# actionml/universal-recommender

Measured on NVIDIA H100. Metric: CCO train events/sec to indicator model, higher is better.
Workload: dtype int32+f64

## Files before the change

### universal_recommender_b200/csrc/cco_api.cu

```cuda
#include <cuda_runtime.h>
#include <dlfcn.h>
#include <stdarg.h>
#include <stdio.h>
#include <stdlib.h>
#include <string.h>

#include <algorithm>
#include <cmath>
#include <functional>
#include <cub/cub.cuh>
#include <nvtx3/nvToolsExt.h>
#include <condition_variable>
#include <mutex>
#include <string>
#include <thread>
#include <unordered_map>
#include <vector>

#include "../../include/cco_b200.h"
#include "cco_kernels.cuh"
#include "cco_sampler.cuh"
#include "cco_format.cuh"
#include "cco_strings.cuh"
#include "cco_json.cuh"
// ... 150 lines not shown
      return pinned[best].p;
    }
    void *p = nullptr;
    size_t cap = (bytes + (1u << 20) - 1) & ~((size_t)(1u << 20) - 1);
    if (cudaHostAlloc(&p, cap, cudaHostAllocPortable) != cudaSuccess) return nullptr;
    pinned.push_back({p, cap, true});
    return p;
  }
  void pinned_put(void *p) {
    std::lock_guard<std::mutex> lk(mu);
    if (arena && (unsigned char *)p >= arena && (unsigned char *)p < arena + arena_bytes) {
      if (--arena_live <= 0) { arena_live = 0; arena_used = 0; }
      return;
    }
    for (auto &b : pinned)
      if (b.p == p) b.used = false;
  }
};

struct ResultMat {
  int64_t row_begin = 0, row_end = 0;
  int32_t n_cols = 0;
  int64_t *row_ptr = nullptr;
  int32_t *col = nullptr;
  double *llr = nullptr;
  int32_t *cnt = nullptr;
};
struct cco_dataset {
  cco_ctx *ctx = nullptr;
  int n_mats = 0;
  long long n_users = 0;
  long long row_base = 0, n_local = 0;
  std::vector<long long> n_cols, nnz;
  std::vector<long long *> rp;
  std::vector<int32_t *> col;
  std::vector<void *> rp_alloc, col_alloc;
  std::vector<long long> block_cap;
  std::vector<long long> q_lo, q_hi;
  std::vector<cudaEvent_t> ready;
  bool h2d_pending = false;
  bool validated = false;
  bool whole = false;
  float ms_h2d = 0;
  std::vector<cco_dictionary_t> dicts;
};

struct cco_result {
  cco_ctx *ctx = nullptr;
  std::vector<ResultMat> mats;
  cco_stats_t stats;
};

namespace cco {

struct Arena {
  cudaStream_t s;
  cco_ctx *c;
  std::vector<void *> ptrs;
  static constexpr size_t kSlabMax = 8u << 20, kSlabBytes = 64u << 20;
  explicit Arena(cudaStream_t st, cco_ctx *ctx = nullptr) : s(st), c(ctx && !ctx->slab_busy ? ctx : nullptr) {
    if (c) {
      c->slab_busy = true;
      c->slab_idx = 0;
      c->slab_off = 0;
    }
  }
  ~Arena() {
    for (void *p : ptrs) cudaFreeAsync(p, s);
    if (c) c->slab_busy = false;
  }
  void *bump(size_t bytes) {
    bytes = (bytes + 255) & ~(size_t)255;
    while (true) {
      if (c->slab_idx < c->slabs.size()) {
        cco_ctx::Slab &sl = c->slabs[c->slab_idx];
        if (c->slab_off + bytes <= sl.cap) {
          void *p = sl.p + c->slab_off;
          c->slab_off += bytes;
          return p;
        }
        ++c->slab_idx;
        c->slab_off = 0;
        continue;
      }
      void *p = nullptr;
      if (cudaMalloc(&p, kSlabBytes) != cudaSuccess) return nullptr;
      c->slabs.push_back({(unsigned char *)p, kSlabBytes});
    }
  }
  template <typename T>
  int alloc(T **out, size_t n) {
    void *p = nullptr;
    size_t bytes = std::max<size_t>(n * sizeof(T), 16);
    if (c && bytes <= kSlabMax) {
      p = bump(bytes);
      if (!p) return set_error(CCO_E_OOM, "cudaMalloc(scratch slab) failed");
      *out = (T *)p;
      return CCO_OK;
    }
    cudaError_t e = cudaMallocAsync(&p, bytes, s);
    if (e != cudaSuccess) return set_error(CCO_E_OOM, "cudaMallocAsync(%zu bytes): %s", bytes, cudaGetErrorString(e));
    ptrs.push_back(p);
    *out = (T *)p;
    return CCO_OK;
  }
  void take(void *p) {
    for (size_t i = 0; i < ptrs.size(); ++i)
      if (ptrs[i] == p) {
        ptrs.erase(ptrs.begin() + i);
        return;
      }
  }
  void release(void *p) {
    for (size_t i = 0; i < ptrs.size(); ++i)
      if (ptrs[i] == p) {
        cudaFreeAsync(p, s);
        ptrs.erase(ptrs.begin() + i);
        return;
      }
  }
};
static int pooled_event(cco_ctx *c, bool timing, cudaEvent_t *out) {
  std::vector<cudaEvent_t> &pool = timing ? c->ev_timing : c->ev_plain;
  size_t &used = timing ? c->ev_timing_used : c->ev_plain_used;
  if (used == pool.size()) {
    cudaEvent_t e;
    CK(timing ? cudaEventCreate(&e) : cudaEventCreateWithFlags(&e, cudaEventDisableTiming));
    pool.push_back(e);
  }
  *out = pool[used++];
  return CCO_OK;
}

static inline void nvtx_push(const char *name) { nvtxRangePushA(name); }
static inline void nvtx_pop() { nvtxRangePop(); }

static inline int grid_for(long long work_items, int block, int sm_count, int waves = 8) {
  long long g = (work_items + block - 1) / block;
  long long cap = (long long)sm_count * waves;
  if (g > cap) g = cap;
  if (g < 1) g = 1;
  return (int)g;
}

constexpr size_t kMailBytes = 1 << 16;
static int mail_fetch(cco_ctx *c, void *dst_host, const void *src_dev, size_t n) {
  size_t off = (c->mail_used + 7) & ~(size_t)7;
  if (off + n > kMailBytes) return set_error(CCO_E_CUDA, "internal: mailbox overflow");
  k_mail_bytes<<<1, 128, 0, c->stream>>>(c->mail_d + off, (const unsigned char *)src_dev, (int)n);
  c->mail_pending.push_back({dst_host, off, n, c->mail_group});
  c->mail_used = off + n;
  return CCO_OK;
}
static int mail_close(cco_ctx *c, int *group) {
  const int g = c->mail_group;
  while ((int)c->mail_ev.size() <= g) {
    cudaEvent_t e;
    CK(cudaEventCreateWithFlags(&e, cudaEventDisableTiming));
    c->mail_ev.push_back(e);
  }
  CK(cudaEventRecord(c->mail_ev[g], c->stream));
  c->mail_group = g + 1;
  if (group) *group = g;
  return CCO_OK;
}
static int mail_wait_group(cco_ctx *c, int g) {
  CK(cudaEventSynchronize(c->mail_ev[g]));
  CK(cudaGetLastError());
  for (auto &m : c->mail_pending)
    if (m.group == g) memcpy(m.dst, c->mail_h + m.off, m.n);
  return CCO_OK;
}
static void mail_reset(cco_ctx *c) {
  c->mail_pending.clear();
  c->mail_used = 0;
  c->mail_group = 0;
}
static int mail_wait(cco_ctx *c) {
  int g = 0;
  CKR(mail_close(c, &g));
  return mail_wait_group(c, g);
}

struct DevRaw {
  long long n_rows = 0;
  long long row_base = 0;
  int32_t n_cols = 0;
  long long nnz = 0;
  long long nnz_cap = 0;
  long long q_base = 0;
  long long *rp = nullptr;
  int32_t *col = nullptr;
};
struct DevMat {
  long long n_rows = 0;
  int32_t n_cols = 0;
  uint32_t *rp = nullptr;
  int32_t *col = nullptr;
  int32_t *marg = nullptr;
};

template <typename T>
static int exclusive_sum(cco_ctx *c, Arena &ar, const T *in, T *out, long long n, cudaStream_t on = nullptr) {
  if (!on) on = c->stream;
  size_t tb = 0;
  CK(cub::DeviceScan::ExclusiveSum(nullptr, tb, in, out, n, on));
  void *tmp;
  CKR(ar.alloc((char **)&tmp, tb));
  CK(cub::DeviceScan::ExclusiveSum(tmp, tb, in, out, n, on));
  ar.release(tmp);
  return CCO_OK;
}
template <typename K, typename V>
static int sort_pairs(cco_ctx *c, Arena &ar, long long n, K **k, V **v, int bits) {
  cudaStream_t s = c->stream;
  K *k1;
  V *v1;
  CKR(ar.alloc(&k1, std::max<long long>(n, 1)));
  CKR(ar.alloc(&v1, std::max<long long>(n, 1)));
  cub::DoubleBuffer<K> kb(*k, k1);
  cub::DoubleBuffer<V> vb(*v, v1);
  size_t tbytes = 0;
  CK(cub::DeviceRadixSort::SortPairs(nullptr, tbytes, kb, vb, n, 0, bits, s));
  void *tmp;
  CKR(ar.alloc((char **)&tmp, tbytes));
  CK(cub::DeviceRadixSort::SortPairs(tmp, tbytes, kb, vb, n, 0, bits, s));
  c->launches++;
  ar.release(tmp);
  ar.release(kb.Alternate());
  ar.release(vb.Alternate());
  *k = kb.Current();
  *v = vb.Current();
  return CCO_OK;
}
static int bits_for(long long n) {
  int b = 1;
  while ((1LL << b) < n) ++b;
  return b;
}

static int canonicalize_device(cco_ctx *c, Arena &ar, DevRaw &m) {
  if (m.nnz == 0) return CCO_OK;
  unsigned long long *k0, *k1;
  CKR(ar.alloc(&k0, m.nnz));
  CKR(ar.alloc(&k1, m.nnz));
  k_expand_keys<<<grid_for(m.n_rows * kSG, 256, c->sm_count), 256, 0, c->stream>>>(m.n_rows, m.rp, m.col, k0);
  c->launches++;
  int row_bits = 1;
  while ((1LL << row_bits) < m.n_rows) ++row_bits;
  cub::DoubleBuffer<unsigned long long> db(k0, k1);
  size_t tb = 0;
  CK(cub::DeviceRadixSort::SortKeys(nullptr, tb, db, m.nnz, 0, 32 + row_bits, c->stream));
  void *tmp;
  CKR(ar.alloc((char **)&tmp, tb));
  CK(cub::DeviceRadixSort::SortKeys(tmp, tb, db, m.nnz, 0, 32 + row_bits, c->stream));
  ar.release(tmp);
  unsigned long long *sorted = db.Current(), *other = db.Alternate();
  uint32_t *flag, *pos;
  CKR(ar.alloc(&flag, m.nnz + 1));
  CKR(ar.alloc(&pos, m.nnz + 1));
  CK(cudaMemsetAsync(flag + m.nnz, 0, 4, c->stream));
  k_unique_flags<<<grid_for(m.nnz, 256, c->sm_count), 256, 0, c->stream>>>(m.nnz, sorted, flag);
  c->launches++;
  CKR(exclusive_sum(c, ar, flag, pos, m.nnz + 1));
  uint32_t n_unique = 0;
  CK(cudaMemcpyAsync(&n_unique, pos + m.nnz, 4, cudaMemcpyDeviceToHost, c->stream));
  k_unique_scatter<<<grid_for(m.nnz, 256, c->sm_count), 256, 0, c->stream>>>(m.nnz, sorted, flag, pos, other, m.col + m.q_base);
  CK(cudaStreamSynchronize(c->stream));
  k_rowptr_from_keys<<<grid_for(m.n_rows + 1, 256, c->sm_count), 256, 0, c->stream>>>(m.n_rows, n_unique, other, m.rp);
  c->launches += 2;
  m.col += m.q_base;
  m.q_base = 0;
  m.nnz = n_unique;
  CK(cudaGetLastError());
  ar.release(flag);
  ar.release(pos);
  ar.release(k0);
  ar.release(k1);
  return CCO_OK;
}

struct HeavyRows {
  int32_t *list = nullptr;
  int *n = nullptr;
};
static int list_heavy_rows(cco_ctx *c, Arena &ar, const DevRaw &raw, HeavyRows *h) {
  CKR(ar.alloc(&h->list, std::max<long long>(raw.n_rows, 1)));
  CKR(ar.alloc(&h->n, 1));
  CK(cudaMemsetAsync(h->n, 0, 4, c->stream));
  if (raw.n_rows > 0) {
    k_list_heavy_rows<<<grid_for(raw.n_rows, 256, c->sm_count), 256, 0, c->stream>>>(raw.n_rows, raw.rp, h->list, h->n);
    c->launches++;
  }
  return CCO_OK;
}
static void launch_check(cco_ctx *c, const DevRaw &raw, const HeavyRows &h, int *flags) {
  if (raw.n_rows <= 0) return;
  const long long q_lo = raw.q_base, q_hi = raw.q_base + raw.nnz;
  k_check_rows<kSG><<<grid_for(raw.n_rows * kSG, 256, c->sm_count), 256, 0, c->stream>>>(raw.n_rows, raw.n_cols, raw.rp, raw.col, q_lo, q_hi,
                                                                                       nullptr, nullptr, flags);
  k_check_rows<32><<<c->sm_count * 4, 256, 0, c->stream>>>(raw.n_rows, raw.n_cols, raw.rp, raw.col, q_lo, q_hi, h.list, h.n, flags);
  c->launches += 2;
}
struct SampleScratch {
  unsigned long long *col_thr = nullptr;
  uint8_t *keep = nullptr;
};
static int sample_scratch(cco_ctx *c, Arena &ar, const DevRaw &raw, const int32_t *raw_counts, int32_t m, SampleScratch *sc) {
  CKR(ar.alloc(&sc->col_thr, std::max<int32_t>(raw.n_cols, 1)));
  CKR(ar.alloc(&sc->keep, std::max<long long>(raw.nnz, 1)));
  if (raw.n_cols > 0) {
    k_col_thresholds<<<grid_for(raw.n_cols, 256, c->sm_count, 4), 256, 0, c->stream>>>(raw.n_cols, raw_counts, m, sc->col_thr);
    c->launches++;
  }
  return CCO_OK;
}
static void launch_count(cco_ctx *c, const DevRaw &raw, const SampleScratch &sc, int32_t m, int32_t seed, uint32_t flags, const int *bad,
                         uint32_t *kept, int32_t *new_counts) {
  if (raw.n_rows <= 0 || raw.nnz <= 0) return;
  const long long q_lo = raw.q_base, q_hi = raw.q_base + raw.nnz;
  const long long n_chunks = (raw.nnz + kSampleChunk - 1) / kSampleChunk;
  k_sample_count<<<grid_for(n_chunks * 32, 256, c->sm_count), 256, 0, c->stream>>>(raw.n_rows, raw.row_base, raw.rp, raw.col, raw.n_cols, q_lo, q_hi,
                                                                                  sc.col_thr, m, seed, flags, bad, kept, new_counts, sc.keep);
  c->launches++;
}
static int launch_write(cco_ctx *c, Arena &ar, const DevRaw &raw, const SampleScratch &sc, int32_t *dst) {
  if (raw.n_rows <= 0 || raw.nnz <= 0) return CCO_OK;
  long long *n_sel;
  CKR(ar.alloc(&n_sel, 1));
  size_t tb = 0;
  CK(cub::DeviceSelect::Flagged(nullptr, tb, raw.col + raw.q_base, sc.keep, dst, n_sel, (long long)raw.nnz, c->stream));
  void *tmp;
  CKR(ar.alloc((char **)&tmp, tb));
  CK(cub::DeviceSelect::Flagged(tmp, tb, raw.col + raw.q_base, sc.keep, dst, n_sel, (long long)raw.nnz, c->stream));
  ar.release(tmp);
  c->launches += 2;
  return CCO_OK;
}

constexpr int kHistCopies = 16;
static int count_raw_columns(cco_ctx *c, const std::vector<DevRaw> &raw, const std::vector<long long> &col_off, const cudaEvent_t *ready,
                             int *verdict, int32_t *counts) {
  cudaStream_t s = c->stream;
  const int n_mats = (int)raw.size();
  const long long total_cols = col_off[n_mats];
  const long long copy_stride = std::max<long long>(total_cols, 1);
  for (int i = 0; i < n_mats; ++i) {
    if (ready) CK(cudaStreamWaitEvent(s, ready[i], 0));
    if (raw[i].n_rows == 0) continue;
    int *v = verdict ? verdict + 2 * i : nullptr;
    if (v) {
      k_check_row_ptr<<<grid_for(raw[i].n_rows, 256, c->sm_count), 256, 0, s>>>(raw[i].n_rows, raw[i].rp, raw[i].q_base, raw[i].q_base + raw[i].nnz, v);
      c->launches++;
    }
    if (raw[i].nnz > 0) {
      k_col_histogram_flat<true><<<grid_for(raw[i].nnz, 256, c->sm_count), 256, 0, s>>>(raw[i].nnz, raw[i].col + raw[i].q_base, raw[i].n_cols,
                                                                                       counts + col_off[i], kHistCopies, copy_stride, v);
      c->launches++;
    }
  }
  if (total_cols > 0) {
    k_sum_copies<<<grid_for(total_cols, 256, c->sm_count), 256, 0, s>>>(total_cols, kHistCopies, copy_stride, counts);
    c->launches++;
  }
  return CCO_OK;
}

static int downsample_device(cco_ctx *c, Arena &ar, const DevRaw &raw, const int *bad, const int32_t *raw_counts, int32_t m,
                             int32_t seed, uint32_t flags, DevMat *out) {
  out->n_rows = raw.n_rows;
  out->n_cols = raw.n_cols;
  uint32_t *kept;
  CKR(ar.alloc(&kept, raw.n_rows + 1));
  CKR(ar.alloc(&out->rp, raw.n_rows + 1));
  if (!out->marg) CKR(ar.alloc(&out->marg, std::max<int32_t>(raw.n_cols, 1)));
  CKR(ar.alloc(&out->col, std::max<long long>(raw.nnz, 1)));
  CK(cudaMemsetAsync(out->marg, 0, sizeof(int32_t) * std::max<int32_t>(raw.n_cols, 1), c->stream));
  CK(cudaMemsetAsync(kept, 0, sizeof(uint32_t) * ((size_t)raw.n_rows + 1), c->stream));
  SampleScratch sc;
  CKR(sample_scratch(c, ar, raw, raw_counts, m, &sc));
  launch_count(c, raw, sc, m, seed, flags, bad, kept, out->marg);
  CKR(exclusive_sum(c, ar, kept, out->rp, raw.n_rows + 1));
  CKR(launch_write(c, ar, raw, sc, out->col));
  CK(cudaGetLastError());
  ar.release(kept);
  ar.release(sc.col_thr);
  ar.release(sc.keep);
  return CCO_OK;
}

static int nccl_check(int rc, const char *what) {
  if (rc != 0) return set_error(CCO_E_NCCL, "%s: %s", what, g_nccl.GetErrorString(rc));
  return CCO_OK;
}

static int downsample_sharded_all(cco_ctx *c, Arena &ar, const std::vector<DevRaw> &raw, const int *d_check ,
                                  const std::vector<long long> &block_cap,
                                  long long U, const int32_t *raw_counts, int32_t *marg_all, const std::vector<long long> &col_off,
                                  const cco_indicator_params_t *params, int32_t seed, uint32_t flags, std::vector<DevMat> &dm,
                                  cudaEvent_t *stage_ev ) {
  cudaStream_t s = c->stream;
  const int W = c->world, r = c->rank, n_mats = (int)raw.size();
  const long long S = (U + W - 1) / W;
  const long long row_base = raw[0].row_base;
  std::vector<uint32_t *> kept(n_mats, nullptr);
  std::vector<SampleScratch> sc(n_mats);
  for (int i = 0; i < n_mats; ++i) {
    DevMat *out = &dm[i];
    out->n_rows = U;
    out->n_cols = raw[i].n_cols;
    out->marg = marg_all + col_off[i];
    CKR(ar.alloc(&kept[i], (size_t)(W * S + 1)));
    CKR(ar.alloc(&out->rp, U + 1));
    CK(cudaMemsetAsync(kept[i], 0, sizeof(uint32_t) * (size_t)(W * S + 1), s));
    CKR(sample_scratch(c, ar, raw[i], raw_counts + col_off[i], params[i].max_interactions, &sc[i]));
    launch_count(c, raw[i], sc[i], params[i].max_interactions, seed, flags, d_check + 2 * i, kept[i], out->marg);
  }
  CK(cudaEventRecord(stage_ev[0], s));
  if (S > 0) {
    g_nccl.GroupStart();
    for (int i = 0; i < n_mats; ++i) {
      int rc = g_nccl.AllGather(kept[i] + (size_t)r * S, kept[i], (size_t)S, kNcclUint32, c->comm, s);
      if (rc != 0) { g_nccl.GroupEnd(); return nccl_check(rc, "ncclAllGather(kept counts)"); }
    }
    CKR(nccl_check(g_nccl.GroupEnd(), "ncclGroupEnd(kept counts)"));
  }
  if (col_off[n_mats] > 0)
    CKR(nccl_check(g_nccl.AllReduce(marg_all, marg_all, (size_t)col_off[n_mats], kNcclInt32, kNcclSum, c->comm, s), "ncclAllReduce(marginals)"));
  std::vector<int32_t *> gathered(n_mats, nullptr);
  std::vector<uint32_t> edge((size_t)n_mats * (W + 1), 0);
  for (int i = 0; i < n_mats; ++i) {
    CKR(exclusive_sum(c, ar, kept[i], dm[i].rp, U + 1));
    ar.release(kept[i]);
    for (int q = 0; q <= W; ++q) CKR(mail_fetch(c, &edge[(size_t)i * (W + 1) + q], dm[i].rp + std::min<long long>((long long)q * S, U), 4));
  }
  CK(cudaEventRecord(stage_ev[1], s));
  CKR(mail_wait(c));
  std::vector<long long> cap(n_mats, 0);
  for (int i = 0; i < n_mats; ++i) {
    for (int q = 0; q < W; ++q) cap[i] = std::max<long long>(cap[i], (long long)edge[(size_t)i * (W + 1) + q + 1] - edge[(size_t)i * (W + 1) + q]);
    CKR(ar.alloc(&dm[i].col, std::max<long long>(edge[(size_t)i * (W + 1) + W], 1)));
    if (cap[i] == 0) continue;
    CKR(ar.alloc(&gathered[i], (size_t)(cap[i] * W)));
    CKR(launch_write(c, ar, raw[i], sc[i], gathered[i] + (size_t)r * cap[i]));
    ar.release(sc[i].col_thr);
    ar.release(sc[i].keep);
  }
  CK(cudaEventRecord(stage_ev[2], s));
  g_nccl.GroupStart();
  for (int i = 0; i < n_mats; ++i) {
    if (!gathered[i]) continue;
    int rc = g_nccl.AllGather(gathered[i] + (size_t)r * cap[i], gathered[i], (size_t)cap[i], kNcclInt32, c->comm, s);
    if (rc != 0) { g_nccl.GroupEnd(); return nccl_check(rc, "ncclAllGather(column blocks)"); }
  }
  CKR(nccl_check(g_nccl.GroupEnd(), "ncclGroupEnd(column blocks)"));
  for (int i = 0; i < n_mats; ++i) {
    if (!gathered[i]) continue;
    dim3 grid((unsigned)std::max(1, std::min(c->sm_count * 8 / W, 1024)), (unsigned)W);
    k_pack_blocks<<<grid, 256, 0, s>>>(W, S, U, cap[i], dm[i].rp, gathered[i], dm[i].col);
    c->launches++;
    ar.release(gathered[i]);
  }
  CK(cudaEventRecord(stage_ev[3], s));
  CK(cudaGetLastError());
  return CCO_OK;
}


struct BinCfg {
  int group;
  int slots;
  int cap;
  int cbuf;
  int caux, keep_max, final_max;
  bool dense;
  bool bitmap;
  int bm_words;
  size_t region;
  size_t smem;
  int ctas_per_sm;
};

static int next_pow2(int x) {
  int p = 1;
  while (p < x) p <<= 1;
  return p;
}

template <int GROUP>
static int launch_rows_t(cco_ctx *c, const RowArgs &a, BinCfg &cfg, cudaStream_t st) {
  constexpr int CTA = GROUP == 32 ? 64 : GROUP;
  int occ = 1;
  void (*kern)(const RowArgs) = cfg.dense ? k_rows<GROUP, true> : k_rows<GROUP, false>;
  if constexpr (GROUP == 512 || GROUP == 256)
    if (cfg.bitmap) kern = k_rows<GROUP, false, true>;
  CK(cudaFuncSetAttribute(kern, cudaFuncAttributeMaxDynamicSharedMemorySize, (int)cfg.smem));
  CK(cudaOccupancyMaxActiveBlocksPerMultiprocessor(&occ, kern, CTA, cfg.smem));
  kern<<<c->sm_count * std::max(occ, 1) * 4, CTA, cfg.smem, st>>>(a);
  cfg.ctas_per_sm = occ;
  c->launches++;
  CK(cudaGetLastError());
  return CCO_OK;
}
static int launch_rows(cco_ctx *c, const RowArgs &a, BinCfg &cfg, cudaStream_t st) {
  switch (cfg.group) {
    case 1024: return launch_rows_t<1024>(c, a, cfg, st);
    case 512: return launch_rows_t<512>(c, a, cfg, st);
    case 256: return launch_rows_t<256>(c, a, cfg, st);
    case 128: return launch_rows_t<128>(c, a, cfg, st);
    case 32: return launch_rows_t<32>(c, a, cfg, st);
  }
  return set_error(CCO_E_INVALID_ARG, "internal: bad bin config");
}

static BinCfg make_cfg(cco_ctx *c, int group, int want_slots, int top_k, int n_cols_b) {
  BinCfg f;
  const int groups = group == 32 ? 2 : 1;
  f.group = group;
  f.final_max = next_pow2(top_k);
  f.cbuf = next_pow2(top_k + std::max(group, 128) + (group == 32 ? 64 : 0));
  if (group == 32 && top_k + 32 <= 96) f.cbuf = 128;
  f.keep_max = std::max(f.final_max, (f.cbuf - group) / 2);
  f.caux = group == 32 ? 0 : f.keep_max;
  size_t fixed = (size_t)(f.cbuf + f.caux) * 16 + 2 * 256 + 512 + 1024 + (size_t)(group / 32) * 256;
  size_t avail = (c->smem_optin - 1024) / groups;
  int max_slots = (int)((avail - fixed) / 4) & ~1023;
  f.slots = std::min(want_slots, max_slots);
  f.cap = f.slots / 2;
  f.dense = n_cols_b <= f.slots;
  f.bitmap = false;
  f.bm_words = 0;
  f.region = (fixed + (size_t)f.slots * 4 + 15) & ~(size_t)15;
  f.smem = f.region * groups;
  f.ctas_per_sm = 1;
  return f;
}

static bool use_bitmap(BinCfg &f, uint32_t max_w, int top_k, int n_cols_b) {
  if (f.dense || (f.group != 512 && f.group != 256)) return false;
  const long long seg = 32LL * (f.group / 32);
  const long long rep = (std::max<long long>(max_w, 64) + seg - 1) / seg * seg;
  const long long bm = ((long long)n_cols_b + 31) / 32;
  if (rep + bm + top_k > f.slots) return false;
  f.bitmap = true;
  f.slots = (int)rep;
  f.bm_words = (int)bm;
  return true;
}

static double llr_error_bound(long long n_users) {
  const double n = (double)n_users;
  return n > 1.0 ? std::ldexp(n * std::log(n), -47) : 0.0;
}
static bool cut_exact(long long n_users, int32_t max_marg_a, int32_t max_marg_b) {
  const double n = (double)n_users, r = (double)max_marg_a, c = (double)max_marg_b;
  if (r <= 0.0 || c <= 0.0) return true;
  double g = 2.0 / std::min(r * c, 0.5 * n);
  const double d = n - c - r + 1.0;
  if (d > 0.0) g = std::max(g, 2.0 * (1.0 / c - (r - 1.0) / d));
  return g > 2.0 * llr_error_bound(n_users);
}

struct IndicatorState {
  int mail_group = -1;
  long long rec[7] = {0, 0, 0, 0, 0, 0, 0};
  cudaEvent_t packed = nullptr;
  long long *out_ptr = nullptr;
  int32_t *p_col = nullptr, *p_cnt = nullptr;
  double *p_llr = nullptr;
  int32_t n_items_a = 0, n_cols_b = 0;
  bool emit_all = false;
};

static int enqueue_indicator(cco_ctx *c, Arena &ar, const uint32_t *at_ptr, const int32_t *at_users, int32_t n_items_a,
                             const int32_t *marg_a, int32_t max_marg_a, int32_t max_marg_b, const DevMat &B, long long n_users,
                             bool self, const cco_indicator_params_t &prm, uint32_t flags, bool emit_all, cudaEvent_t inputs_ready,
                             cudaEvent_t ev_begin, cudaEvent_t ev_end, IndicatorState *st) {
  cudaStream_t s = c->stream;
  const int32_t n_cols_b = B.n_cols;
  const int rank = c->rank, world = c->world;
  st->n_items_a = n_items_a;
  st->n_cols_b = n_cols_b;
  st->emit_all = emit_all;
  uint32_t *row_work, *masked, *sorted_work;
  unsigned long long *work64;
  long long *work_prefix;
  int32_t *ids, *rows_sorted, *d_pb = nullptr;
  size_t sort_tb = 0, order_tb = 0;
  if (n_items_a > 0)
    CK(cub::DeviceRadixSort::SortPairsDescending(nullptr, sort_tb, (const uint32_t *)nullptr, (uint32_t *)nullptr, (const int32_t *)nullptr,
                                                 (int32_t *)nullptr, n_items_a, 0, 32, s));
  int cb_bits = 1;
  while ((1LL << cb_bits) <= (long long)max_marg_b) ++cb_bits;
  cub::DoubleBuffer<uint32_t> order_cb(nullptr, nullptr);
  cub::DoubleBuffer<int32_t> order_id(nullptr, nullptr);
  if (n_cols_b > 0) CK(cub::DeviceRadixSort::SortPairs(nullptr, order_tb, order_cb, order_id, n_cols_b, 0, cb_bits, s));
  const bool beside = inputs_ready && ar.c && ((size_t)n_items_a + 1) * 8 <= Arena::kSlabMax && sort_tb <= Arena::kSlabMax &&
                      (size_t)n_cols_b * 4 <= Arena::kSlabMax && order_tb <= Arena::kSlabMax &&
                      ((size_t)max_marg_b + 2) * 4 <= Arena::kSlabMax;
  cudaStream_t ss = beside ? c->sched_stream : s;
  if (beside) CK(cudaStreamWaitEvent(ss, inputs_ready, 0));
  CKR(ar.alloc(&row_work, n_items_a + 1));
  CKR(ar.alloc(&masked, n_items_a + 1));
  CKR(ar.alloc(&work64, n_items_a + 1));
  CKR(ar.alloc(&work_prefix, n_items_a + 1));
  CKR(ar.alloc(&ids, n_items_a + 1));
  CKR(ar.alloc(&sorted_work, n_items_a + 1));
  CKR(ar.alloc(&rows_sorted, n_items_a + 1));
  CK(cudaMemsetAsync(work64 + n_items_a, 0, 8, ss));
  k_row_work<<<grid_for((long long)n_items_a * kSG, 256, c->sm_count), 256, 0, ss>>>(n_items_a, at_ptr, at_users, B.rp,
                                                                                  row_work, work64, ids, nullptr);
  c->launches++;
  CKR(exclusive_sum(c, ar, (const long long *)work64, work_prefix, (long long)n_items_a + 1, ss));
  if (world > 1) {
    CKR(ar.alloc(&d_pb, world + 1));
    k_partition_rows<<<1, ((world + 1 + 31) / 32) * 32, 0, ss>>>(work_prefix, n_items_a, world, d_pb);
    c->launches++;
  }
  k_mask_work<<<grid_for(n_items_a, 256, c->sm_count), 256, 0, ss>>>(n_items_a, row_work, d_pb, rank, masked);
  c->launches++;
  if (n_items_a > 0) {
    void *tmp;
    CKR(ar.alloc((char **)&tmp, sort_tb));
    CK(cub::DeviceRadixSort::SortPairsDescending(tmp, sort_tb, masked, sorted_work, ids, rows_sorted, n_items_a, 0, 32, ss));
    ar.release(tmp);
  }
  const int k_eff = emit_all ? 1 : prm.top_k;
  const bool warp_ok = k_eff + 32 <= 256;
  struct BinSpec { int group, slots; uint32_t max_w; };
  std::vector<BinSpec> spec = {{1024, 1 << 20, 0xffffffffu}, {1024, 1 << 20, 0xffffffffu}, {512, 16384, 8192u}, {256, 8192, 4096u}};
  if (warp_ok) {
    spec.push_back({128, 4096, 2048u});
    spec.push_back({32, 2048, 1024u});
    spec.push_back({32, 1024, 512u});
    spec.push_back({32, 512, 256u});
  } else {
    spec.push_back({128, 4096, 2048u});
  }
  const int kBins = (int)spec.size();
  std::vector<BinCfg> cfgs(kBins);
  for (int b = 0; b < kBins; ++b) cfgs[b] = make_cfg(c, spec[b].group, spec[b].slots, k_eff, n_cols_b);
  BinCfg &cfgL = cfgs[1];
  int key_bits = 1;
  while (((1LL << key_bits) - 1) <= (long long)n_cols_b) ++key_bits;
  int count_bits = 32 - key_bits;
  const long long k11_max = std::min<long long>(max_marg_a, max_marg_b);
  if (count_bits < 1 || k11_max >= (1LL << count_bits))
    return set_error(CCO_E_UNSUPPORTED,
                     "co-occurrence counts up to %lld over %d columns do not fit the packed 32-bit accumulator word "
                     "(key %d bits + count %d bits): lower maxItemsPerUser/maxEventsPerEventType for this event type "
                     "(\"Limits\" in include/cco_b200.h)", k11_max, n_cols_b, key_bits, count_bits);
  std::vector<uint32_t> h_thr(kBins);
  for (int b = 0; b < kBins; ++b) {
    const BinCfg &f = cfgs[std::min(b + 1, kBins - 1)];
    uint32_t lim = b + 1 < kBins ? spec[b + 1].max_w : 0u;
    if (b + 1 < kBins && !f.dense) lim = std::min<uint32_t>(lim, (uint32_t)f.cap);
    h_thr[b] = lim;
    if (b > 0) h_thr[b] = std::min(h_thr[b], h_thr[b - 1]);
  }
  const bool bitmap_ok = !emit_all && cut_exact(n_users, max_marg_a, max_marg_b) &&
                         2ull * (unsigned long long)std::max(max_marg_a, 0) * (unsigned long long)std::max(max_marg_b, 0) <
                             (unsigned long long)n_users;
  for (int b = 1; b < kBins && bitmap_ok; ++b) use_bitmap(cfgs[b], h_thr[b - 1], k_eff, n_cols_b);
  int32_t *d_bounds;
  CKR(ar.alloc(&d_bounds, kBins + 3));
  BinThresholds bt;
  memset(&bt, 0, sizeof bt);
  for (int b = 0; b < kBins; ++b) bt.t[b] = h_thr[b];
  k_bin_bounds<<<1, 32, 0, ss>>>(n_items_a, sorted_work, kBins, bt, d_bounds);
  c->launches++;
  int32_t *key_of_col, *first_key_of_cb, *order_id0, *order_id1;
  uint32_t *order_cb0, *order_cb1;
  const int32_t n_order = std::max<int32_t>(n_cols_b, 1);
  CKR(ar.alloc(&key_of_col, n_order));
  CKR(ar.alloc(&first_key_of_cb, (size_t)max_marg_b + 2));
  CKR(ar.alloc(&order_cb0, n_order));
  CKR(ar.alloc(&order_cb1, n_order));
  CKR(ar.alloc(&order_id0, n_order));
  CKR(ar.alloc(&order_id1, n_order));
  order_cb = cub::DoubleBuffer<uint32_t>(order_cb0, order_cb1);
  order_id = cub::DoubleBuffer<int32_t>(order_id0, order_id1);
  if (n_cols_b > 0) {
    k_col_order_init<<<grid_for(n_cols_b, 256, c->sm_count, 4), 256, 0, ss>>>(n_cols_b, B.marg, order_cb0, order_id0);
    void *tmp;
    CKR(ar.alloc((char **)&tmp, order_tb));
    CK(cub::DeviceRadixSort::SortPairs(tmp, order_tb, order_cb, order_id, n_cols_b, 0, cb_bits, ss));
    ar.release(tmp);
    k_col_order<<<grid_for(n_cols_b, 256, c->sm_count, 4), 256, 0, ss>>>(n_cols_b, max_marg_b, order_cb.Current(), order_id.Current(),
                                                                        key_of_col, first_key_of_cb);
    k_relabel_cols<<<c->sm_count * 8, 256, 0, ss>>>(B.rp + B.n_rows, key_of_col, B.col);
    c->launches += 3;
  }
  const int32_t *marg_key = reinterpret_cast<const int32_t *>(order_cb.Current()), *col_of_key = order_id.Current();
  if (beside) {
    cudaEvent_t scheduled;
    CKR(pooled_event(c, false, &scheduled));
    CK(cudaEventRecord(scheduled, ss));
    CK(cudaStreamWaitEvent(s, scheduled, 0));
  }
  ColTerm *col_terms;
  CKR(ar.alloc(&col_terms, std::max<int32_t>(n_cols_b, 1)));
  if (n_cols_b > 0) {
    k_col_terms<<<grid_for(n_cols_b, 256, c->sm_count, 4), 256, 0, s>>>(n_cols_b, marg_key, col_of_key, n_users, flags, col_terms);
    c->launches++;
  }
  int32_t stride = emit_all ? n_cols_b : std::min<int32_t>(prm.top_k, n_cols_b);
  if (stride < 1) stride = 1;
  int32_t *o_col, *o_cnt, *o_len;
  double *o_llr = nullptr;
  unsigned long long *d_distinct;
  int *d_err;
  size_t cells = (size_t)std::max(n_items_a, 1) * stride;
  CKR(ar.alloc(&o_col, cells));
  CKR(ar.alloc(&o_cnt, cells));
  if (!emit_all) CKR(ar.alloc(&o_llr, cells));
  CKR(ar.alloc(&o_len, n_items_a + 1));
  CKR(ar.alloc(&d_distinct, 2));
  CKR(ar.alloc(&d_err, 1));
  CK(cudaMemsetAsync(o_len, 0, sizeof(int32_t) * ((size_t)n_items_a + 1), s));
  CK(cudaMemsetAsync(d_distinct, 0, 16, s));
  CK(cudaMemsetAsync(d_err, 0, 4, s));
  RowArgs a;
  memset(&a, 0, sizeof a);
  a.at_ptr = at_ptr;
  a.at_users = at_users;
  a.b_ptr = B.rp;
  a.b_col = B.col;
  a.marg_a = marg_a;
  a.marg_b = marg_key;
  a.key_of_col = key_of_col;
  a.first_key_of_cb = first_key_of_cb;
  a.key_shift = 0;
  while (((long long)std::max(n_cols_b - 1, 0) >> a.key_shift) >= kCutBins) ++a.key_shift;
  a.max_marg_b = max_marg_b;
  a.col_terms = col_terms;
  a.rows_sorted = rows_sorted;
  a.row_work = row_work;
  a.bin_bounds = d_bounds;
  a.n_cols_b = n_cols_b;
  a.n_users = n_users;
  a.self = self ? 1 : 0;
  a.top_k = k_eff;
  a.has_min_llr = prm.has_min_llr;
  a.min_llr = prm.min_llr;
  a.cut_ok = cut_exact(n_users, max_marg_a, max_marg_b) ? 1 : 0;
  a.llr_eps2 = 2.0 * llr_error_bound(n_users);
  a.flags = flags;
  a.count_bits = count_bits;
  a.out_stride = stride;
  a.out_col = o_col;
  a.out_llr = o_llr;
  a.out_cnt = o_cnt;
  a.out_len = o_len;
  a.stat_distinct = d_distinct;
  a.stat_evaluated = d_distinct + 1;
  a.err_flag = d_err;
  a.emit_all = emit_all ? 1 : 0;
  if (ev_begin) CK(cudaEventRecord(ev_begin, s));
  if (n_items_a > 0) {
    CK(cudaEventRecord(c->bin_ev[8], s));
    for (int b = 0; b < kBins; ++b) {
      if (b == 0 && cfgL.dense) continue;
      RowArgs ab = a;
      ab.bin = b;
// ... 57 lines not shown
  io->distinct = st->rec[4];
  io->evaluated = st->rec[5];
  if (st->rec[6]) return set_error(CCO_E_CUDA, "internal: shared-memory hash table overflow");
  const int32_t n_my = hi - lo;
  cudaStream_t cs = c->copy_stream;
  CK(cudaStreamWaitEvent(cs, st->packed, 0));
  GroupShared *gs = c->gshared;
  int64_t *h_rp;
  int32_t *h_col, *h_cnt = nullptr;
  double *h_llr = nullptr;
  long long base = 0;
  if (gs) {
    {
      std::lock_guard<std::mutex> lk(gs->mu);
      gs->totals[c->rank] = total;
    }
    gs->barrier();
    long long grand = 0;
    for (int q = 0; q < gs->world; ++q) {
      if (q < c->rank) base += gs->totals[q];
      grand += gs->totals[q];
    }
    ResultMat &mm = gs->merged->mats[index];
    if (c->rank == 0) {
      cco_ctx *owner = gs->merged->ctx;
      mm.row_begin = 0;
      mm.row_end = st->n_items_a;
      mm.n_cols = st->n_cols_b;
      mm.row_ptr = (int64_t *)owner->pinned_get(sizeof(int64_t) * ((size_t)st->n_items_a + 1));
      mm.col = (int32_t *)owner->pinned_get(sizeof(int32_t) * (size_t)std::max<long long>(grand, 1));
      if (st->p_cnt) mm.cnt = (int32_t *)owner->pinned_get(sizeof(int32_t) * (size_t)std::max<long long>(grand, 1));
      if (st->p_llr) mm.llr = (double *)owner->pinned_get(sizeof(double) * (size_t)std::max<long long>(grand, 1));
    }
    gs->barrier();
    if (!mm.row_ptr || !mm.col || (st->p_cnt && !mm.cnt) || (st->p_llr && !mm.llr)) return set_error(CCO_E_OOM, "pinned host allocation failed");
    h_rp = mm.row_ptr + lo;
    h_col = mm.col + base;
    h_cnt = mm.cnt ? mm.cnt + base : nullptr;
    h_llr = mm.llr ? mm.llr + base : nullptr;
    if (base != 0 && n_my >= 0) {
      k_add_i64<<<grid_for((long long)n_my + 1, 256, c->sm_count, 2), 256, 0, cs>>>((long long)n_my + 1, base, st->out_ptr + lo);
      c->launches++;
    }
    rm->row_begin = lo;
    rm->row_end = hi;
    rm->n_cols = st->n_cols_b;
  } else {
    rm->row_begin = lo;
    rm->row_end = hi;
    rm->n_cols = st->n_cols_b;
    rm->row_ptr = (int64_t *)c->pinned_get(sizeof(int64_t) * ((size_t)n_my + 1));
    rm->col = (int32_t *)c->pinned_get(sizeof(int32_t) * (size_t)std::max<long long>(total, 1));
    if (st->p_cnt) rm->cnt = (int32_t *)c->pinned_get(sizeof(int32_t) * (size_t)std::max<long long>(total, 1));
    if (st->p_llr) rm->llr = (double *)c->pinned_get(sizeof(double) * (size_t)std::max<long long>(total, 1));
    if (!rm->row_ptr || !rm->col || (st->p_cnt && !rm->cnt) || (st->p_llr && !rm->llr))
      return set_error(CCO_E_OOM, "pinned host allocation failed");
    h_rp = rm->row_ptr;
    h_col = rm->col;
    h_cnt = rm->cnt;
    h_llr = rm->llr;
  }
  CK(cudaMemcpyAsync(h_rp, st->out_ptr + lo, sizeof(int64_t) * ((size_t)n_my + 1), cudaMemcpyDeviceToHost, cs));
  if (total > 0 && !(flags & CCO_FLAG_RESULT_ON_DEVICE)) {
    CK(cudaMemcpyAsync(h_col, st->p_col, sizeof(int32_t) * (size_t)total, cudaMemcpyDeviceToHost, cs));
    if (h_cnt) CK(cudaMemcpyAsync(h_cnt, st->p_cnt, sizeof(int32_t) * (size_t)total, cudaMemcpyDeviceToHost, cs));
    if (h_llr) CK(cudaMemcpyAsync(h_llr, st->p_llr, sizeof(double) * (size_t)total, cudaMemcpyDeviceToHost, cs));
  }
  return CCO_OK;
}

static int validate_host(int32_t n_mats, const cco_csr_t *mats, const cco_indicator_params_t *params) {
  if (n_mats < 1 || !mats || !params) return set_error(CCO_E_INVALID_ARG, "need at least the primary matrix and its params");
  for (int i = 0; i < n_mats; ++i) {
    const cco_csr_t &m = mats[i];
    if (!m.row_ptr) return set_error(CCO_E_INVALID_ARG, "matrix %d: null row_ptr", i);
    if (m.n_rows < 0 || m.n_rows >= 0x7fffffffLL) return set_error(CCO_E_INVALID_ARG, "matrix %d: n_rows out of range", i);
    if (m.n_cols < 0 || m.n_cols >= 0x7ffffffe) return set_error(CCO_E_INVALID_ARG, "matrix %d: n_cols out of range", i);
    if (m.n_rows != mats[0].n_rows)
      return set_error(CCO_E_SHAPE_MISMATCH, "matrix %d has %lld rows, the primary has %lld: all event types share the user dictionary",
                       i, (long long)m.n_rows, (long long)mats[0].n_rows);
    if (m.row_ptr[0] != 0) return set_error(CCO_E_INVALID_ARG, "matrix %d: row_ptr[0] != 0", i);
    long long nnz = m.row_ptr[m.n_rows];
    if (nnz < 0 || nnz >= 0xffffffffLL) return set_error(CCO_E_UNSUPPORTED, "matrix %d: nnz %lld outside [0, 2^32)", i, nnz);
    if (nnz > 0 && !m.col_idx) return set_error(CCO_E_INVALID_ARG, "matrix %d: null col_idx", i);
    if (params[i].max_interactions < 1) return set_error(CCO_E_INVALID_ARG, "matrix %d: max_interactions must be >= 1", i);
    if (params[i].top_k < 1) return set_error(CCO_E_INVALID_ARG, "matrix %d: top_k must be >= 1", i);
    if (params[i].top_k > CCO_MAX_TOP_K)
      return set_error(CCO_E_UNSUPPORTED, "matrix %d: top_k %d > CCO_MAX_TOP_K (%d)", i, params[i].top_k, CCO_MAX_TOP_K);
    if (params[i].has_min_llr && params[i].min_llr != params[i].min_llr)
      return set_error(CCO_E_INVALID_ARG, "matrix %d: min_llr is NaN", i);
  }
  return CCO_OK;
}

static inline void user_block(long long U, int W, int r, long long *lo, long long *hi) {
  const long long S = (U + W - 1) / W;
  *lo = std::min<long long>((long long)r * S, U);
  *hi = std::min<long long>(*lo + S, U);
}

static void dataset_release(cco_dataset *d) {
  if (!d) return;
  cudaSetDevice(d->ctx->device);
  for (auto p : d->rp_alloc)
    if (p) cudaFreeAsync(p, d->ctx->stream);
  for (auto p : d->col_alloc)
    if (p) cudaFreeAsync(p, d->ctx->stream);
  for (auto e : d->ready)
    if (e) cudaEventDestroy(e);
  for (auto &dc : d->dicts) {
    if (dc.offsets) d->ctx->pinned_put((void *)dc.offsets);
    if (dc.bytes) d->ctx->pinned_put((void *)dc.bytes);
  }
  delete d;
}

static int dataset_validate(cco_ctx *c, cco_dataset *d, bool canonicalise) {
  cudaStream_t s = c->stream;
  const int n_mats = d->n_mats;
  Arena ar(s);
  int *d_flags;
  CKR(ar.alloc(&d_flags, 2 * n_mats));
  CK(cudaMemsetAsync(d_flags, 0, sizeof(int) * 2 * n_mats, s));
  for (int i = 0; i < n_mats; ++i) {
    CK(cudaStreamWaitEvent(s, d->ready[i], 0));
    if (d->n_local == 0) continue;
    DevRaw r;
    r.n_rows = d->n_local;
    r.n_cols = (int32_t)d->n_cols[i];
    r.q_base = d->q_lo[i];
    r.nnz = d->q_hi[i] - d->q_lo[i];
    r.rp = d->rp[i];
    r.col = d->col[i];
    HeavyRows hv;
    CKR(list_heavy_rows(c, ar, r, &hv));
    launch_check(c, r, hv, d_flags + 2 * i);
  }
  if (c->world > 1)
    CKR(nccl_check(g_nccl.AllReduce(d_flags, d_flags, (size_t)(2 * n_mats), kNcclInt32, kNcclMax, c->comm, s), "ncclAllReduce(check flags)"));
  std::vector<int> h(2 * n_mats);
  CK(cudaMemcpyAsync(h.data(), d_flags, sizeof(int) * 2 * n_mats, cudaMemcpyDeviceToHost, s));
  CK(cudaStreamSynchronize(s));
  CK(cudaGetLastError());
  for (int i = 0; i < n_mats; ++i)
    if (h[2 * i]) return set_error(CCO_E_INVALID_ARG, "matrix %d: row_ptr not monotone or column index out of [0, n_cols)", i);
  if (canonicalise)
    for (int i = 0; i < n_mats; ++i)
      if (h[2 * i + 1] && d->n_local > 0) {
        DevRaw r;
        r.n_rows = d->n_local;
        r.row_base = d->row_base;
        r.n_cols = (int32_t)d->n_cols[i];
        r.q_base = d->q_lo[i];
        r.nnz = d->q_hi[i] - d->q_lo[i];
        r.rp = d->rp[i];
        r.col = d->col[i];
        CKR(canonicalize_device(c, ar, r));
        d->col[i] = r.col;
        d->q_lo[i] = 0;
        d->q_hi[i] = r.nnz;
        if (c->world == 1) d->nnz[i] = r.nnz;
      }
  CK(cudaStreamSynchronize(s));
  d->validated = canonicalise;
  return CCO_OK;
}

static int dataset_upload(cco_ctx *c, int32_t n_mats, const cco_csr_t *mats, uint32_t flags, cco_dataset **out, bool async = false) {
  CK(cudaSetDevice(c->device));
  cudaStream_t s = c->stream;
  cco_dataset *d = new cco_dataset();
  d->ctx = c;
  d->n_mats = n_mats;
  d->n_users = mats[0].n_rows;
  long long u_lo, u_hi;
  user_block(d->n_users, c->world, c->rank, &u_lo, &u_hi);
  d->row_base = u_lo;
  d->n_local = u_hi - u_lo;
  d->whole = c->world == 1;
  d->rp.assign(n_mats, nullptr);
  d->col.assign(n_mats, nullptr);
  d->rp_alloc.assign(n_mats, nullptr);
  d->col_alloc.assign(n_mats, nullptr);
  d->n_cols.assign(n_mats, 0);
  d->nnz.assign(n_mats, 0);
  d->block_cap.assign(n_mats, 0);
  d->q_lo.assign(n_mats, 0);
  d->q_hi.assign(n_mats, 0);
  d->ready.assign(n_mats, nullptr);
  struct G {
    cco_dataset *d;
    bool ok = false;
    ~G() {
      if (!ok) dataset_release(d);
    }
  } g{d};
  cudaStream_t cs = c->copy_stream;
  for (int i = 0; i < n_mats; ++i) {
    const cco_csr_t &m = mats[i];
    d->n_cols[i] = m.n_cols;
    d->nnz[i] = m.row_ptr[m.n_rows];
    for (int q = 0; q < c->world; ++q) {
      long long a0, a1;
      user_block(d->n_users, c->world, q, &a0, &a1);
      d->block_cap[i] = std::max<long long>(d->block_cap[i], m.row_ptr[a1] - m.row_ptr[a0]);
    }
    const long long q0 = m.row_ptr[u_lo], q1 = m.row_ptr[u_hi];
    d->q_lo[i] = q0;
    d->q_hi[i] = q1;
    void *p = nullptr;
    cudaError_t e = cudaMallocAsync(&p, sizeof(int64_t) * ((size_t)d->n_local + 1), s);
    if (e != cudaSuccess) return set_error(CCO_E_OOM, "cudaMallocAsync row_ptr: %s", cudaGetErrorString(e));
    d->rp_alloc[i] = p;
    d->rp[i] = (long long *)p;
    e = cudaMallocAsync(&p, sizeof(int32_t) * (size_t)std::max<long long>(q1 - q0, 4), s);
    if (e != cudaSuccess) return set_error(CCO_E_OOM, "cudaMallocAsync col_idx: %s", cudaGetErrorString(e));
    d->col_alloc[i] = p;
    d->col[i] = (int32_t *)p - q0;
    CK(cudaEventCreateWithFlags(&d->ready[i], cudaEventDisableTiming));
  }
  CK(cudaEventRecord(c->copy_ev[0], s));
  CK(cudaStreamWaitEvent(cs, c->copy_ev[0], 0));
  CK(cudaEventRecord(c->ev[6], cs));
  for (int i = 0; i < n_mats; ++i) {
    const cco_csr_t &m = mats[i];
    const long long q0 = m.row_ptr[u_lo], q1 = m.row_ptr[u_hi];
    CK(cudaMemcpyAsync(d->rp_alloc[i], m.row_ptr + u_lo, sizeof(int64_t) * ((size_t)d->n_local + 1), cudaMemcpyHostToDevice, cs));
    if (q1 > q0)
      CK(cudaMemcpyAsync(d->col_alloc[i], m.col_idx + q0, sizeof(int32_t) * (size_t)(q1 - q0), cudaMemcpyHostToDevice, cs));
    CK(cudaEventRecord(d->ready[i], cs));
  }
  CK(cudaEventRecord(c->ev[7], cs));
  if (async && (flags & CCO_FLAG_ASSUME_CANONICAL)) {
    d->h2d_pending = true;
    g.ok = true;
    *out = d;
    return CCO_OK;
  }
  CKR(dataset_validate(c, d, !(flags & CCO_FLAG_ASSUME_CANONICAL)));
  CK(cudaEventElapsedTime(&d->ms_h2d, c->ev[6], c->ev[7]));
  g.ok = true;
  *out = d;
  return CCO_OK;
}

static int train_dataset(cco_ctx *c, const cco_dataset *ds, const cco_indicator_params_t *params, int32_t seed, uint32_t flags,
                         cco_result **out) {
  CK(cudaSetDevice(c->device));
  cudaStream_t s = c->stream;
  const int n_mats = ds->n_mats;
  mail_reset(c);
  c->ev_timing_used = c->ev_plain_used = 0;
  Arena ar(s, c);
  struct CopyJoin {
    cco_ctx *c;
    ~CopyJoin() {
      cudaStreamSynchronize(c->copy_stream);
      cudaStreamSynchronize(c->sched_stream);
    }
  } copy_join{c};
  cco_result *res = new cco_result();
  res->ctx = c;
  res->mats.resize(n_mats);
  memset(&res->stats, 0, sizeof res->stats);
  struct Guard {
    cco_result *r;
    bool ok = false;
    ~Guard() {
      if (!ok) cco_result_free(r);
    }
  } guard{res};
  std::vector<IndicatorState> ist(n_mats);
  for (auto &x : ist) CKR(pooled_event(c, false, &x.packed));
  cco_stats_t &st = res->stats;
  st.n_mats = n_mats;
  st.n_users = ds->n_users;
  st.ms_h2d = ds->ms_h2d;
  const bool h2d_pending = ds->h2d_pending;
  const long long n_users = ds->n_users;
  std::vector<DevRaw> raw(n_mats);
  for (int i = 0; i < n_mats; ++i) {
    raw[i].n_rows = ds->n_local;
    raw[i].row_base = ds->row_base;
    raw[i].n_cols = (int32_t)ds->n_cols[i];
    raw[i].q_base = ds->q_lo[i];
    raw[i].nnz = ds->q_hi[i] - ds->q_lo[i];
    raw[i].nnz_cap = ds->nnz[i];
    raw[i].rp = ds->rp[i];
    raw[i].col = ds->col[i];
    st.nnz_in_total += ds->nnz[i];
  }
  CK(cudaEventRecord(c->ev[1], s));
  nvtx_push("cco:prepare");
  std::vector<cudaEvent_t> sev(8, nullptr);
  for (auto &e : sev) CKR(pooled_event(c, true, &e));
  auto mark = [&](int k) { return cudaEventRecord(sev[k], s); };
  long long total_cols = 0;
  std::vector<long long> col_off(n_mats + 1, 0);
  for (int i = 0; i < n_mats; ++i) {
    col_off[i] = total_cols;
    total_cols += raw[i].n_cols;
  }
  col_off[n_mats] = total_cols;
  const long long copy_stride = std::max<long long>(total_cols, 1);
  int32_t *raw_counts, *marg_all;
  int *d_check;
  CKR(ar.alloc(&raw_counts, (size_t)copy_stride * kHistCopies));
  CKR(ar.alloc(&marg_all, (size_t)copy_stride));
  CKR(ar.alloc(&d_check, 2 * n_mats));
  CK(cudaMemsetAsync(raw_counts, 0, sizeof(int32_t) * (size_t)copy_stride * kHistCopies, s));
  CK(cudaMemsetAsync(marg_all, 0, sizeof(int32_t) * (size_t)copy_stride, s));
  CK(cudaMemsetAsync(d_check, 0, sizeof(int) * 2 * n_mats, s));
  CKR(count_raw_columns(c, raw, col_off, ds->ready.data(), ds->validated ? nullptr : d_check, raw_counts));
  CK(mark(0));
  if (c->world > 1) {
    if (total_cols > 0)
      CKR(nccl_check(g_nccl.AllReduce(raw_counts, raw_counts, (size_t)total_cols, kNcclInt32, kNcclSum, c->comm, s), "ncclAllReduce(raw counts)"));
    CKR(nccl_check(g_nccl.AllReduce(d_check, d_check, (size_t)(2 * n_mats), kNcclInt32, kNcclMax, c->comm, s), "ncclAllReduce(check flags)"));
  }
  CK(mark(1));
  std::vector<DevMat> dm(n_mats);
  if (c->world > 1) {
    CKR(downsample_sharded_all(c, ar, raw, d_check, ds->block_cap, n_users, raw_counts, marg_all, col_off, params, seed, flags, dm, &sev[2]));
  } else {
    for (int i = 0; i < n_mats; ++i) {
      dm[i].marg = marg_all + col_off[i];
      CKR(downsample_device(c, ar, raw[i], d_check + 2 * i, raw_counts + col_off[i], params[i].max_interactions, seed, flags, &dm[i]));
    }
    CK(mark(2));
    CK(mark(3));
    CK(mark(4));
    CK(mark(5));
  }
  const int32_t n_items_a = dm[0].n_cols;
  uint32_t *at_ptr, *cursor;
  int32_t *at_users, *d_max;
  CKR(ar.alloc(&at_ptr, n_items_a + 1));
  CKR(ar.alloc(&cursor, n_items_a + 1));
  CKR(ar.alloc(&d_max, n_mats));
  CKR(ar.alloc(&at_users, std::max<long long>(ds->nnz[0], 1)));
  CK(cudaMemsetAsync(d_max, 0, 4 * (size_t)n_mats, s));
  {
    uint32_t *marg_pad;
    CKR(ar.alloc(&marg_pad, n_items_a + 1));
    CK(cudaMemcpyAsync(marg_pad, dm[0].marg, sizeof(int32_t) * (size_t)n_items_a, cudaMemcpyDeviceToDevice, s));
    CK(cudaMemsetAsync(marg_pad + n_items_a, 0, 4, s));
    CKR(exclusive_sum(c, ar, marg_pad, at_ptr, (long long)n_items_a + 1));
    ar.release(marg_pad);
  }
  CK(cudaMemcpyAsync(cursor, at_ptr, sizeof(uint32_t) * ((size_t)n_items_a + 1), cudaMemcpyDeviceToDevice, s));
  k_transpose_scatter<<<grid_for(n_users * kSG, 256, c->sm_count), 256, 0, s>>>(n_users, dm[0].rp, dm[0].col, cursor, at_users);
  c->launches++;
  for (int i = 0; i < n_mats; ++i)
    if (dm[i].n_cols > 0) {
      k_max_i32<<<grid_for(dm[i].n_cols, 256, c->sm_count, 2), 256, 0, s>>>(dm[i].n_cols, dm[i].marg, d_max + i);
      c->launches++;
    }
  std::vector<int32_t> max_marg(n_mats, 0);
  std::vector<uint32_t> h_nnz(n_mats);
  std::vector<int> h_check(2 * n_mats, 0);
  CKR(mail_fetch(c, max_marg.data(), d_max, 4 * (size_t)n_mats));
  CKR(mail_fetch(c, h_check.data(), d_check, sizeof(int) * 2 * (size_t)n_mats));
  for (int i = 0; i < n_mats; ++i) CKR(mail_fetch(c, &h_nnz[i], dm[i].rp + n_users, 4));
  CK(mark(6));
  CK(cudaEventRecord(c->ev[2], s));
  nvtx_pop();
  CKR(mail_wait(c));
  for (int i = 0; i < n_mats; ++i)
    if (h_check[2 * i]) return set_error(CCO_E_INVALID_ARG, "matrix %d: row_ptr not monotone or column index out of [0, n_cols)", i);
  for (int i = 0; i < n_mats && i < 16; ++i) st.nnz_downsampled[i] = h_nnz[i];

  std::vector<IndicatorOut> io(n_mats);
  std::vector<cudaEvent_t> ev_rows(2 * n_mats, nullptr);
  for (auto &e : ev_rows) CKR(pooled_event(c, true, &e));
  for (int i = 0; i < n_mats; ++i) {
    nvtx_push("cco:indicator");
    CKR(enqueue_indicator(c, ar, at_ptr, at_users, n_items_a, dm[0].marg, max_marg[0], max_marg[i], dm[i], n_users, i == 0, params[i],
                          flags, false, c->ev[2], ev_rows[2 * i], ev_rows[2 * i + 1], &ist[i]));
    nvtx_pop();
    if (i > 0) CKR(finish_indicator(c, &ist[i - 1], flags, i - 1, &res->mats[i - 1], &io[i - 1]));
  }
  CKR(finish_indicator(c, &ist[n_mats - 1], flags, n_mats - 1, &res->mats[n_mats - 1], &io[n_mats - 1]));
  CK(cudaEventRecord(c->copy_ev[1], c->copy_stream));
  CK(cudaStreamWaitEvent(s, c->copy_ev[1], 0));
  CK(cudaEventRecord(c->ev[3], s));
  CK(cudaStreamSynchronize(s));
  CK(cudaStreamSynchronize(c->copy_stream));
  for (int i = 0; i < n_mats && i < 16; ++i) {
    st.products[i] = io[i].products;
    st.distinct_cells[i] = io[i].distinct;
    st.llr_evaluated[i] = io[i].evaluated;
    st.out_nnz[i] = io[i].nnz;
    CK(cudaEventElapsedTime(&st.ms_indicator[i], ev_rows[2 * i], ev_rows[2 * i + 1]));
  }
  if (h2d_pending) CK(cudaEventElapsedTime(&st.ms_h2d, c->ev[6], c->ev[7]));
  CK(cudaEventElapsedTime(&st.ms_prep_stage[0], c->ev[1], sev[0]));
  for (int k = 1; k <= 6; ++k) CK(cudaEventElapsedTime(&st.ms_prep_stage[k], sev[k - 1], sev[k]));
  CK(cudaEventElapsedTime(&st.ms_prepare, c->ev[1], c->ev[2]));
  CK(cudaEventElapsedTime(&st.ms_cooccurrence, c->ev[2], c->ev[3]));
  CK(cudaEventElapsedTime(&st.ms_total, c->ev[1], c->ev[3]));
  if (!h2d_pending) st.ms_total += st.ms_h2d;
  st.n_kernel_launches = c->launches;
  guard.ok = true;
  *out = res;
  return CCO_OK;
}

static int train_impl(cco_ctx *c, int32_t n_mats, const cco_csr_t *mats, const cco_indicator_params_t *params, int32_t seed,
                      uint32_t flags, cco_result **out) {
  c->launches = 0;
  cco_dataset *ds = nullptr;
  CKR(dataset_upload(c, n_mats, mats, flags, &ds, true));
  int rc = train_dataset(c, ds, params, seed, flags, out);
  cudaStreamSynchronize(c->copy_stream);
  dataset_release(ds);
  return rc;
}

static int train_group(cco_ctx *leader, int32_t n_mats, const cco_csr_t *mats, const cco_indicator_params_t *params, int32_t seed,
                       uint32_t flags, cco_result **out) {
  const int W = (int)leader->members.size();
  GroupShared *gs = leader->members[0]->gshared;
  cco_result *merged = new cco_result();
  merged->ctx = leader;
  merged->mats.resize(n_mats);
  memset(&merged->stats, 0, sizeof merged->stats);
  gs->merged = merged;
  gs->totals.assign(W, 0);
  gs->status = CCO_OK;
  gs->err[0] = 0;
  std::vector<cco_result *> part(W, nullptr);
  std::vector<std::thread> th;
  for (int r = 0; r < W; ++r)
    th.emplace_back([&, r]() {
      int rc = train_impl(leader->members[r], n_mats, mats, params, seed, flags, &part[r]);
      if (rc != CCO_OK) {
        std::lock_guard<std::mutex> lk(gs->mu);
        if (gs->status == CCO_OK) {
          gs->status = rc;
          snprintf(gs->err, sizeof gs->err, "GPU %d: %s", leader->members[r]->device, cco_last_error());
        }
      }
    });
  for (auto &t : th) t.join();
  gs->merged = nullptr;
  if (gs->status != CCO_OK) {
    for (auto p : part)
      if (p) cco_result_free(p);
    cco_result_free(merged);
    return set_error(gs->status, "%s", gs->err);
  }
  cco_stats_t &st = merged->stats;
  st = part[0]->stats;
  for (int r = 1; r < W; ++r) {
    const cco_stats_t &p = part[r]->stats;
    for (int i = 0; i < 16; ++i) {
      st.products[i] += p.products[i];
      st.distinct_cells[i] += p.distinct_cells[i];
      st.out_nnz[i] += p.out_nnz[i];
      st.llr_evaluated[i] += p.llr_evaluated[i];
      st.ms_indicator[i] = std::max(st.ms_indicator[i], p.ms_indicator[i]);
    }
    st.ms_h2d = std::max(st.ms_h2d, p.ms_h2d);
    st.ms_prepare = std::max(st.ms_prepare, p.ms_prepare);
    st.ms_cooccurrence = std::max(st.ms_cooccurrence, p.ms_cooccurrence);
    st.ms_total = std::max(st.ms_total, p.ms_total);
    st.n_kernel_launches += p.n_kernel_launches;
  }
  for (auto p : part) cco_result_free(p);
  *out = merged;
  return CCO_OK;
}

}

extern "C" {

int cco_abi_version(void) { return CCO_ABI_VERSION; }
const char *cco_last_error(void) { return g_err; }
const char *cco_status_string(int s) {
  switch (s) {
    case CCO_OK: return "ok";
    case CCO_E_INVALID_ARG: return "invalid argument";
    case CCO_E_CUDA: return "CUDA error";
    case CCO_E_NCCL: return "NCCL error";
    case CCO_E_OOM: return "out of memory";
    case CCO_E_SHAPE_MISMATCH: return "shape mismatch";
    case CCO_E_UNSUPPORTED: return "unsupported";
  }
  return "unknown";
}

int cco_device_count(void) {
  int n = 0;
  cudaError_t e = cudaGetDeviceCount(&n);
  if (e != cudaSuccess) return set_error(CCO_E_CUDA, "cudaGetDeviceCount: %s", cudaGetErrorString(e));
  int ok = 0;
  for (int i = 0; i < n; ++i) {
    cudaDeviceProp p;
    if (cudaGetDeviceProperties(&p, i) == cudaSuccess && p.major == 9 && p.minor == 0) ++ok;
  }
  return ok;
}

int cco_nccl_unique_id(unsigned char out[128]) {
  if (!out) return set_error(CCO_E_INVALID_ARG, "null output");
  CKR(load_nccl());
  ncclUniqueId id;
  int r = g_nccl.GetUniqueId(&id);
  if (r != 0) return set_error(CCO_E_NCCL, "ncclGetUniqueId: %s", g_nccl.GetErrorString(r));
  memcpy(out, id.internal, 128);
  return CCO_OK;
}

static int ctx_init_device(cco_ctx *c) {
  CK(cudaSetDevice(c->device));
  CK(cudaStreamCreateWithFlags(&c->stream, cudaStreamNonBlocking));
  CK(cudaStreamCreateWithFlags(&c->copy_stream, cudaStreamNonBlocking));
  for (auto &ev : c->ev) CK(cudaEventCreate(&ev));
  for (auto &ev : c->tev) CK(cudaEventCreate(&ev));
  for (auto &ev : c->copy_ev) CK(cudaEventCreateWithFlags(&ev, cudaEventDisableTiming));
  for (auto &st : c->bin_stream) CK(cudaStreamCreateWithFlags(&st, cudaStreamNonBlocking));
  int lo_pri = 0, hi_pri = 0;
  CK(cudaDeviceGetStreamPriorityRange(&lo_pri, &hi_pri));
  CK(cudaStreamCreateWithPriority(&c->sched_stream, cudaStreamNonBlocking, hi_pri));
  for (auto &ev : c->bin_ev) CK(cudaEventCreateWithFlags(&ev, cudaEventDisableTiming));
  CK(cudaHostAlloc((void **)&c->mail_h, kMailBytes, cudaHostAllocMapped | cudaHostAllocPortable));
  CK(cudaHostGetDevicePointer((void **)&c->mail_d, c->mail_h, 0));
  cudaMemPool_t pool;
  CK(cudaDeviceGetDefaultMemPool(&pool, c->device));
  uint64_t thr = UINT64_MAX;
  CK(cudaMemPoolSetAttribute(pool, cudaMemPoolAttrReleaseThreshold, &thr));
  return CCO_OK;
}

static int check_device(int device, cudaDeviceProp *p) {
  int n = 0;
  cudaError_t e = cudaGetDeviceCount(&n);
  if (e != cudaSuccess || n == 0)
    return set_error(CCO_E_CUDA, "no CUDA device (%s): this library has no CPU fallback",
                     e != cudaSuccess ? cudaGetErrorString(e) : "device count 0");
  if (device < 0 || device >= n) return set_error(CCO_E_INVALID_ARG, "device %d not in [0,%d)", device, n);
  CK(cudaGetDeviceProperties(p, device));
  if (p->major != 9 || p->minor != 0)
    return set_error(CCO_E_CUDA, "device %d is sm_%d%d; this build contains sm_90a code only", device, p->major, p->minor);
  return CCO_OK;
}

static int create_failed(cco_ctx *c, int st) {
  char keep[sizeof g_err];
  memcpy(keep, g_err, sizeof keep);
  cco_destroy(c);
  memcpy(g_err, keep, sizeof keep);
  return st;
}

int cco_create(const cco_config_t *cfg, cco_ctx_t **out) {
  if (!cfg || !out) return set_error(CCO_E_INVALID_ARG, "null argument");
  if (cfg->world_size < 1 || cfg->rank < 0 || cfg->rank >= cfg->world_size)
    return set_error(CCO_E_INVALID_ARG, "bad rank/world_size %d/%d", cfg->rank, cfg->world_size);
  if (cfg->world_size > 1023) return set_error(CCO_E_UNSUPPORTED, "world_size %d > 1023", cfg->world_size);
  cudaDeviceProp p;
  CKR(check_device(cfg->device, &p));
  if (cfg->world_size > 1 && !cfg->nccl_unique_id) return set_error(CCO_E_INVALID_ARG, "world_size > 1 needs nccl_unique_id");
  cco_ctx *c = new cco_ctx();
  c->device = cfg->device;
  c->rank = cfg->rank;
  c->world = cfg->world_size;
  c->sm_count = p.multiProcessorCount;
  c->smem_optin = p.sharedMemPerBlockOptin;
  auto init = [&]() -> int {
    CKR(ctx_init_device(c));
    if (cfg->result_arena && cfg->result_arena_bytes > 0) {
      CK(cudaHostRegister(cfg->result_arena, cfg->result_arena_bytes, cudaHostRegisterPortable));
      c->arena = (unsigned char *)cfg->result_arena;
      c->arena_bytes = cfg->result_arena_bytes;
      c->arena_registered = true;
    }
    if (c->world > 1) {
      CKR(load_nccl());
      ncclUniqueId id;
      memcpy(id.internal, cfg->nccl_unique_id, 128);
      int rc = g_nccl.CommInitRank(&c->comm, c->world, id, c->rank);
      if (rc != 0) return set_error(CCO_E_NCCL, "ncclCommInitRank: %s", g_nccl.GetErrorString(rc));
    }
    return CCO_OK;
  };
  const int st = init();
  if (st != CCO_OK) return create_failed(c, st);
  *out = c;
  return CCO_OK;
}

int cco_create_group(int32_t n_devices, const int32_t *devices, cco_ctx_t **out) {
  if (!devices || !out || n_devices < 1) return set_error(CCO_E_INVALID_ARG, "bad argument");
  if (n_devices > 1023) return set_error(CCO_E_UNSUPPORTED, "more than 1023 devices");
  std::vector<cudaDeviceProp> props(n_devices);
  for (int r = 0; r < n_devices; ++r) {
    CKR(check_device(devices[r], &props[r]));
    for (int q = 0; q < r; ++q)
      if (devices[q] == devices[r]) return set_error(CCO_E_INVALID_ARG, "device %d listed twice", devices[r]);
  }
  cco_ctx *leader = new cco_ctx();
  leader->device = devices[0];
  leader->world = 1;
  GroupShared *gs = new GroupShared();
  gs->world = n_devices;
  auto init = [&]() -> int {
    std::vector<ncclComm_t> comms(n_devices, nullptr);
    if (n_devices > 1) {
      CKR(load_nccl());
      std::vector<int> devs(devices, devices + n_devices);
      int rc = g_nccl.CommInitAll(comms.data(), n_devices, devs.data());
      if (rc != 0) return set_error(CCO_E_NCCL, "ncclCommInitAll: %s", g_nccl.GetErrorString(rc));
    }
    for (int r = 0; r < n_devices; ++r) {
      cco_ctx *m = new cco_ctx();
      m->device = devices[r];
      m->rank = r;
      m->world = n_devices;
      m->sm_count = props[r].multiProcessorCount;
      m->smem_optin = props[r].sharedMemPerBlockOptin;
      m->comm = comms[r];
      m->gshared = gs;
      leader->members.push_back(m);
      CKR(ctx_init_device(m));
    }
    CK(cudaSetDevice(devices[0]));
    return CCO_OK;
  };
  const int st = init();
  if (st != CCO_OK) {
    if (leader->members.empty()) delete gs;
    return create_failed(leader, st);
  }
  *out = leader;
  return CCO_OK;
}

int cco_destroy(cco_ctx_t *c) {
  if (!c) return CCO_OK;
  if (!c->members.empty()) {
    GroupShared *gs = c->members[0]->gshared;
    for (cco_ctx *m : c->members) {
      m->gshared = nullptr;
      cco_destroy(m);
    }
    c->members.clear();
    delete gs;
  }
  cudaSetDevice(c->device);
  if (c->stream) cudaStreamSynchronize(c->stream);
  if (c->copy_stream) cudaStreamSynchronize(c->copy_stream);
  if (c->comm) g_nccl.CommDestroy(c->comm);
// ... 2541 lines not shown
  log_drop(lg, lg->rline);
  lg->tline = lg->rline = nullptr;
  if (lg->n_prop > 0) {
    mail_reset(c);
    Arena ar(s);
    CKR(event_pad(c, lg->pb, lg->pb_len));
    EvLines ev;
    CKR(event_lines(c, ar, (const uint64_t *)lg->pb, lg->pb_len, false, 0, &ev));
    if (n_prop_dup > 0) CKR(win_drop_property_lines(lg, ar, ev, drop));
    CKR(event_properties(c, ar, lg, ev.L, ev.flag, ev.tm, ev.sb, ev.span, lg->pb, lg->prop_line.data()));
    CK(cudaStreamSynchronize(s));
  }
  log_drop(lg, drop);
  log_drop(lg, lg->pb);
  lg->pb = nullptr;
  lg->prop_line = std::vector<long long>();
  CK(cudaStreamSynchronize(s));
  CK(cudaGetLastError());
  lg->finished = true;
  return CCO_OK;
}

static int log_rankings(const cco_event_log *lg, int32_t n_rank, const cco_log_ranking_t *lr, std::vector<cco_ranking_t> *rk, Streams *ls) {
  if (n_rank < 0 || (n_rank > 0 && !lr)) return set_error(CCO_E_INVALID_ARG, "bad rankings");
  rk->assign((size_t)std::max(n_rank, 0), cco_ranking_t{});
  ls->assign((size_t)std::max(n_rank, 0), {});
  const int NG = (int)lg->n_rank.size();
  for (int k = 0; k < n_rank; ++k) {
    const cco_log_ranking_t &r = lr[k];
    (*rk)[k] = cco_ranking_t{r.name, r.mode, 0, r.start_ms, r.end_ms, nullptr};
    std::vector<int> codes;
    if (r.mode == CCO_POP_RANDOM) {
      for (int g = 0; g < NG; ++g) codes.push_back(g);
    } else {
      if (r.n_event_names < 0 || (r.n_event_names > 0 && !r.event_names)) return set_error(CCO_E_INVALID_ARG, "ranking %d: bad event names", k);
      for (int q = 0; q < r.n_event_names; ++q) {
        if (!r.event_names[q]) return set_error(CCO_E_INVALID_ARG, "ranking %d: null event name", k);
        codes.push_back(lg->code_of(r.event_names[q]));
      }
    }
    for (int g : codes) {
      if (g < 0) continue;
      Stream st;
      st.items.n = lg->n_rank[g];
      st.items.off = (const int64_t *)(lg->ri.off + lg->rank_at[g]);
      st.items.bytes = (const char *)lg->ri.w + lg->ri.boff[g];
      st.items.device = true;
      st.items.base = lg->ri.boff[g];
      st.items.nbytes = lg->ri.boff[g + 1] - lg->ri.boff[g];
      st.time = (const int64_t *)(lg->rtime + lg->rank_at[g]);
      (*ls)[k].push_back(st);
    }
  }
  return CCO_OK;
}
static int log_state(const cco_event_log *lg, bool want_finished) {
  if (lg->fail != CCO_OK) return set_error(CCO_E_INVALID_ARG, "the read of this log failed: %s", lg->fail_msg.c_str());
  if (lg->finished != want_finished)
    return set_error(CCO_E_INVALID_ARG, want_finished ? "the log is not finished (cco_event_log_finish)" : "the log is finished");
  return CCO_OK;
}
static int log_fail(cco_event_log *lg, int rc) {
  if (rc != CCO_OK) {
    lg->fail = rc;
    lg->fail_msg = g_err;
  }
  return rc;
}
}

int cco_event_log_begin(cco_ctx_t *ctx, int64_t chunk_bytes, cco_event_log_t **out) {
  return cco_event_log_begin_window(ctx, chunk_bytes, nullptr, out);
}

int cco_event_log_begin_window(cco_ctx_t *ctx, int64_t chunk_bytes, const cco_event_window_t *w, cco_event_log_t **out) {
  if (!ctx || !out || chunk_bytes < 1) return set_error(CCO_E_INVALID_ARG, "null argument or chunk_bytes < 1");
  *out = nullptr;
  if (w && (w->remove_duplicates != 0 && w->remove_duplicates != 1))
    return set_error(CCO_E_INVALID_ARG, "remove_duplicates is %d, not 0 or 1", (int)w->remove_duplicates);
  if (w && w->reserved != 0) return set_error(CCO_E_INVALID_ARG, "the window's reserved field must be 0");
  if (!ctx->members.empty()) return set_error(CCO_E_UNSUPPORTED, "an event log is resident on one GPU: read it on a per-GPU context");
  CKR(event_log_begin(ctx, chunk_bytes, out));
  if (w) {
    (*out)->cutoff = w->cutoff_ms;
    (*out)->dedup = w->remove_duplicates != 0;
  }
  return CCO_OK;
}

int cco_event_log_window_stats(const cco_event_log_t *lg, int64_t *n_expired, int64_t *n_duplicates) {
  if (!lg || !n_expired || !n_duplicates) return set_error(CCO_E_INVALID_ARG, "null argument");
  CKR(log_state(lg, true));
  *n_expired = lg->n_expired;
  *n_duplicates = lg->n_dup;
  return CCO_OK;
}

int cco_event_log_append(cco_event_log_t *lg, const char *bytes, int64_t len) {
  if (!lg || len < 0 || (len > 0 && !bytes)) return set_error(CCO_E_INVALID_ARG, "null argument or negative length");
  CKR(log_state(lg, false));
  return log_fail(lg, event_log_append(lg, bytes, len));
}

int cco_event_log_finish(cco_event_log_t *lg) {
  if (!lg) return set_error(CCO_E_INVALID_ARG, "null argument");
  CKR(log_state(lg, false));
  return log_fail(lg, event_log_finish(lg));
}

int cco_event_log_read(cco_ctx_t *ctx, const char *bytes, int64_t len, cco_event_log_t **out) {
  if (!ctx || !out || len < 0 || (len > 0 && !bytes)) return set_error(CCO_E_INVALID_ARG, "null argument or negative length");
  *out = nullptr;
  if (!ctx->members.empty()) return set_error(CCO_E_UNSUPPORTED, "an event log is resident on one GPU: read it on a per-GPU context");
  nvtx_push("cco:event_log_read");
  struct Pop { ~Pop() { nvtx_pop(); } } pop;
  cco_event_log *lg = nullptr;
  CKR(event_log_begin(ctx, std::max<int64_t>(len, 1), &lg));
  int rc = event_log_append(lg, bytes, len);
  if (rc == CCO_OK) rc = event_log_finish(lg);
  if (rc != CCO_OK) {
    event_log_release(lg);
    return rc;
  }
  *out = lg;
  return CCO_OK;
}

int cco_event_log_info(const cco_event_log_t *lg, cco_event_log_info_t *out) {
  if (!lg || !out) return set_error(CCO_E_INVALID_ARG, "null argument");
  CKR(log_state(lg, true));
  out->n_lines = lg->n_lines;
  out->names = cco_dictionary_t{(int64_t)lg->n_train.size(), lg->name_off.data(), lg->name_bytes.data()};
  out->n_training = lg->n_train.data();
  out->n_ranking = lg->n_rank.data();
  out->n_property_events = lg->n_prop;
  out->n_property_items = lg->n_prop_items;
  out->n_property_fields = lg->n_prop_fields;
  out->n_ignored = lg->n_ignored;
  return CCO_OK;
}

int cco_event_log_ingest(cco_ctx_t *c, const cco_event_log_t *lg, int32_t n_names, const char *const *names, int32_t min_events_per_user,
                         cco_dataset_t **out) {
  if (!c || !lg || !names || !out || n_names < 1) return set_error(CCO_E_INVALID_ARG, "bad argument");
  *out = nullptr;
  if (!c->members.empty() || lg->ctx != c) return set_error(CCO_E_UNSUPPORTED, "ingest a log on the per-GPU context that read it");
  CKR(log_state(lg, true));
  std::vector<int> codes(n_names);
  for (int t = 0; t < n_names; ++t) {
    if (!names[t]) return set_error(CCO_E_INVALID_ARG, "null event name %d", t);
    codes[t] = lg->code_of(names[t]);
  }
  const StrColumns view = [lg, &codes](Arena &ar, int t, DevStrCol *uc, DevStrCol *ic) -> int {
    const int g = codes[t];
    const long long n = g >= 0 ? lg->n_train[g] : 0;
    *uc = lg->view(lg->tu, g, lg->train_at, n);
    *ic = lg->view(lg->ti, g, lg->train_at, n);
    CKR(ar.alloc(&uc->hash, std::max<long long>(n, 1)));
    CKR(ar.alloc(&ic->hash, std::max<long long>(n, 1)));
    return CCO_OK;
  };
  return ingest_strings_core(c, n_names, view, min_events_per_user, out);
}

namespace cco {
struct LogProps {
  std::vector<const char *> names;
  cco_item_properties_t shell;
  DevProps dev;
};
static void log_props(const cco_event_log *lg, LogProps *p) {
  for (const std::string &f : lg->field_names) p->names.push_back(f.c_str());
  p->shell = cco_item_properties_t{lg->n_triples, nullptr, nullptr, nullptr, nullptr, nullptr, (int32_t)p->names.size(), p->names.data()};
  p->dev.items = KeySection{lg->n_triples, (const int64_t *)lg->p_ioff, (const char *)lg->p_ibytes, true, lg->p_ibytes_n, 0};
  p->dev.field = lg->p_field;
  p->dev.voff = lg->p_voff;
  p->dev.vals = lg->p_vals;
}
}

int cco_format_model_log(cco_ctx_t *ctx, const cco_result_t *res, int32_t n_names, const char *const *names,
                         const cco_dictionary_t *row_ids, const cco_dictionary_t *col_ids, const cco_event_log_t *lg, int32_t n_rankings,
                         const cco_log_ranking_t *rankings, char **out_bytes, int64_t *out_len) {
  if (!ctx || !lg) return set_error(CCO_E_INVALID_ARG, "null argument");
  if (!ctx->members.empty() || lg->ctx != ctx) return set_error(CCO_E_UNSUPPORTED, "format on the per-GPU context that read the log");
  CKR(log_state(lg, true));
  std::vector<cco_ranking_t> rk;
  Streams ls;
  CKR(log_rankings(lg, n_rankings, rankings, &rk, &ls));
  LogProps lp;
  log_props(lg, &lp);
  const bool any = lg->n_triples > 0;
  return format_model(ctx, res, n_names, names, row_ids, col_ids, any ? &lp.shell : nullptr, n_rankings, rk.data(), out_bytes, out_len,
                      "cco:format_model_log", std::move(ls), any ? &lp.dev : nullptr);
}

int cco_rerank_model_log(cco_ctx_t *ctx, const char *body, int64_t body_len, const cco_event_log_t *lg, int32_t n_rankings,
                         const cco_log_ranking_t *rankings, char **out_bytes, int64_t *out_len) {
  if (!ctx || !lg) return set_error(CCO_E_INVALID_ARG, "null argument");
  if (!ctx->members.empty() || lg->ctx != ctx) return set_error(CCO_E_UNSUPPORTED, "rerank on the per-GPU context that read the log");
  CKR(log_state(lg, true));
  std::vector<cco_ranking_t> rk;
  Streams ls;
  CKR(log_rankings(lg, n_rankings, rankings, &rk, &ls));
  LogProps lp;
  log_props(lg, &lp);
  const bool any = lg->n_triples > 0;
  return rerank_model(ctx, body, body_len, any ? &lp.shell : nullptr, n_rankings, rk.data(), out_bytes, out_len, std::move(ls),
                      any ? &lp.dev : nullptr);
}

int cco_event_log_free(cco_event_log_t *lg) {
  event_log_release(lg);
  return CCO_OK;
}

int cco_pop_model(cco_ctx_t *ctx, int32_t mode, int64_t n_events, const int32_t *item, const int64_t *time_ms, int32_t n_items,
                  int64_t start_ms, int64_t end_ms, double *score, unsigned char *present) {
  if (!ctx || n_events < 0 || n_items < 0 || (n_events > 0 && (!item || !time_ms)) || (n_items > 0 && (!score || !present)))
    return set_error(CCO_E_INVALID_ARG, "bad argument");
  if (mode < CCO_POP_POPULAR || mode > CCO_POP_HOT) return set_error(CCO_E_INVALID_ARG, "mode must be CCO_POP_POPULAR, _TRENDING or _HOT");
  if (end_ms < start_ms) return set_error(CCO_E_INVALID_ARG, "end before start (Joda Interval would throw)");
  if (n_items == 0) return CCO_OK;
  cco_ctx *c = ctx->members.empty() ? ctx : ctx->members[0];
  CK(cudaSetDevice(c->device));
  cudaStream_t s = c->stream;
  Arena ar(s);
  nvtx_push("cco:pop_model");
  struct Pop { ~Pop() { nvtx_pop(); } } pop;
  const PopArgs a = pop_args(mode, start_ms, end_ms, n_items);
  int32_t *d_item, *d_counts;
  long long *d_t;
  unsigned long long *d_tot;
  double *d_score;
  unsigned char *d_present;
  CKR(ar.alloc(&d_item, std::max<long long>(n_events, 1)));
  CKR(ar.alloc(&d_t, std::max<long long>(n_events, 1)));
  CKR(ar.alloc(&d_counts, (size_t)a.n_buckets * n_items));
  CKR(ar.alloc(&d_tot, 4));
  CKR(ar.alloc(&d_score, n_items));
  CKR(ar.alloc(&d_present, n_items));
  CK(cudaMemsetAsync(d_counts, 0, sizeof(int32_t) * (size_t)a.n_buckets * n_items, s));
  CK(cudaMemsetAsync(d_tot, 0, 32, s));
  if (n_events > 0) {
    CK(cudaMemcpyAsync(d_item, item, sizeof(int32_t) * (size_t)n_events, cudaMemcpyHostToDevice, s));
    CK(cudaMemcpyAsync(d_t, time_ms, sizeof(int64_t) * (size_t)n_events, cudaMemcpyHostToDevice, s));
    k_pop_count<<<grid_for(n_events, 256, c->sm_count), 256, 0, s>>>(n_events, d_item, d_t, a, d_counts, d_tot);
    c->launches++;
  }
  k_pop_score<double><<<grid_for(n_items, 256, c->sm_count), 256, 0, s>>>(a, mode, d_counts, d_tot, d_score, d_present);
  c->launches++;
  CK(cudaMemcpyAsync(score, d_score, sizeof(double) * (size_t)n_items, cudaMemcpyDeviceToHost, s));
  CK(cudaMemcpyAsync(present, d_present, (size_t)n_items, cudaMemcpyDeviceToHost, s));
  CK(cudaStreamSynchronize(s));
  CK(cudaGetLastError());
  return CCO_OK;
}

void cco_free(void *p) { free(p); }

int cco_debug_llr(cco_ctx_t *c, int64_t n, const int64_t *k11, const int64_t *k12, const int64_t *k21, const int64_t *k22,
                  uint32_t flags, double *out) {
  if (!c || n < 0 || (n > 0 && (!k11 || !k12 || !k21 || !k22 || !out))) return set_error(CCO_E_INVALID_ARG, "bad argument");
  if (n == 0) return CCO_OK;
  for (int64_t i = 0; i < n; ++i)
    if (k11[i] < 0 || k12[i] < 0 || k21[i] < 0 || k22[i] < 0)
      return set_error(CCO_E_INVALID_ARG, "negative count at %lld (Preconditions.checkArgument in LogLikelihood)", (long long)i);
  CK(cudaSetDevice(c->device));
  Arena ar(c->stream);
  long long *d[4];
  double *dout;
  const int64_t *h[4] = {k11, k12, k21, k22};
  for (int j = 0; j < 4; ++j) {
    CKR(ar.alloc(&d[j], n));
    CK(cudaMemcpyAsync(d[j], h[j], sizeof(int64_t) * (size_t)n, cudaMemcpyHostToDevice, c->stream));
  }
  CKR(ar.alloc(&dout, n));
  k_debug_llr<<<(unsigned)((n + 255) / 256), 256, 0, c->stream>>>(n, d[0], d[1], d[2], d[3], flags, dout);
  CK(cudaMemcpyAsync(out, dout, sizeof(double) * (size_t)n, cudaMemcpyDeviceToHost, c->stream));
  CK(cudaStreamSynchronize(c->stream));
  CK(cudaGetLastError());
  return CCO_OK;
}

int cco_debug_downsample(cco_ctx_t *c, const cco_csr_t *m, int32_t max_interactions, int32_t seed, uint32_t flags,
                         int64_t **row_ptr, int32_t **col_idx, int32_t *raw_col_counts, int32_t *new_col_counts) {
  if (!c || !m || !row_ptr || !col_idx) return set_error(CCO_E_INVALID_ARG, "null argument");
  if (c->world != 1 || !c->members.empty()) return set_error(CCO_E_UNSUPPORTED, "debug entries need a single-GPU context");
  cco_indicator_params_t prm = {max_interactions, 1, 0, 0.0};
  CKR(validate_host(1, m, &prm));
  CK(cudaSetDevice(c->device));
  mail_reset(c);
  cco_dataset *ds = nullptr;
  CKR(dataset_upload(c, 1, m, flags, &ds));
  struct DG { cco_dataset *d; ~DG() { dataset_release(d); } } dg{ds};
  Arena ar(c->stream);
  std::vector<DevRaw> raw(1);
  raw[0].n_rows = ds->n_users; raw[0].n_cols = (int32_t)ds->n_cols[0]; raw[0].nnz = ds->nnz[0]; raw[0].nnz_cap = ds->nnz[0];
  raw[0].rp = ds->rp[0]; raw[0].col = ds->col[0];
  const std::vector<long long> col_off = {0, m->n_cols};
  const int32_t width = std::max<int32_t>(m->n_cols, 1);
  int32_t *counts;
  int *d_check;
  CKR(ar.alloc(&counts, (size_t)width * kHistCopies));
  CKR(ar.alloc(&d_check, 2));
  CK(cudaMemsetAsync(counts, 0, sizeof(int32_t) * (size_t)width * kHistCopies, c->stream));
  CK(cudaMemsetAsync(d_check, 0, sizeof(int) * 2, c->stream));
  int *verdict = ds->validated ? nullptr : d_check;
  CKR(count_raw_columns(c, raw, col_off, ds->ready.data(), verdict, counts));
  DevMat dm;
  CKR(downsample_device(c, ar, raw[0], verdict, counts, max_interactions, seed, flags, &dm));
  std::vector<uint32_t> rp32((size_t)m->n_rows + 1);
  int h_check = 0;
  CK(cudaMemcpyAsync(rp32.data(), dm.rp, sizeof(uint32_t) * rp32.size(), cudaMemcpyDeviceToHost, c->stream));
  CK(cudaMemcpyAsync(&h_check, d_check, sizeof(int), cudaMemcpyDeviceToHost, c->stream));
  if (raw_col_counts && m->n_cols > 0)
    CK(cudaMemcpyAsync(raw_col_counts, counts, sizeof(int32_t) * (size_t)m->n_cols, cudaMemcpyDeviceToHost, c->stream));
  if (new_col_counts && m->n_cols > 0)
    CK(cudaMemcpyAsync(new_col_counts, dm.marg, sizeof(int32_t) * (size_t)m->n_cols, cudaMemcpyDeviceToHost, c->stream));
  CK(cudaStreamSynchronize(c->stream));
  CK(cudaGetLastError());
  if (h_check) return set_error(CCO_E_INVALID_ARG, "row_ptr not monotone or column index out of [0, n_cols)");
  size_t nnz = rp32[m->n_rows];
  int64_t *rp = (int64_t *)malloc(sizeof(int64_t) * rp32.size());
  int32_t *ci = (int32_t *)calloc(std::max<size_t>(nnz, 1), sizeof(int32_t));
  if (!rp || !ci) return set_error(CCO_E_OOM, "malloc failed");
  for (size_t i = 0; i < rp32.size(); ++i) rp[i] = rp32[i];
  const size_t n_copy = std::min<size_t>(nnz, (size_t)raw[0].nnz);
  if (n_copy) CK(cudaMemcpy(ci, dm.col, sizeof(int32_t) * n_copy, cudaMemcpyDeviceToHost));
  *row_ptr = rp;
  *col_idx = ci;
  return CCO_OK;
}

int cco_debug_downsample_block(cco_ctx_t *c, const cco_csr_t *m, int64_t row_lo, int64_t row_hi, const int32_t *raw_col_counts,
                               int32_t max_interactions, int32_t seed, uint32_t flags, int64_t *kept_per_row, int32_t **col_idx,
                               int32_t *new_col_counts) {
  if (!c || !m || !col_idx || (m->n_rows > 0 && !kept_per_row) || (m->n_cols > 0 && (!raw_col_counts || !new_col_counts)))
    return set_error(CCO_E_INVALID_ARG, "null argument");
  if (c->world != 1 || !c->members.empty()) return set_error(CCO_E_UNSUPPORTED, "debug entries need a single-GPU context");
  cco_indicator_params_t prm = {max_interactions, 1, 0, 0.0};
  CKR(validate_host(1, m, &prm));
  if (row_lo < 0 || row_hi < row_lo || row_hi > m->n_rows)
    return set_error(CCO_E_INVALID_ARG, "rows [%lld, %lld) outside [0, %lld)", (long long)row_lo, (long long)row_hi, (long long)m->n_rows);
  CK(cudaSetDevice(c->device));
  mail_reset(c);
  cudaStream_t s = c->stream;
  cco_dataset *ds = nullptr;
  CKR(dataset_upload(c, 1, m, flags, &ds));
  struct DG { cco_dataset *d; ~DG() { dataset_release(d); } } dg{ds};
  Arena ar(s);
  const long long U = ds->n_users;
  const int32_t width = std::max<int32_t>(m->n_cols, 1);
  long long q[2] = {0, 0};
  CK(cudaMemcpyAsync(&q[0], ds->rp[0] + row_lo, sizeof(long long), cudaMemcpyDeviceToHost, s));
  CK(cudaMemcpyAsync(&q[1], ds->rp[0] + row_hi, sizeof(long long), cudaMemcpyDeviceToHost, s));
  CK(cudaStreamSynchronize(s));
  DevRaw blk;
  blk.n_rows = row_hi - row_lo;
  blk.row_base = row_lo;
  blk.n_cols = m->n_cols;
  blk.q_base = q[0];
  blk.nnz = q[1] - q[0];
  blk.nnz_cap = ds->nnz[0];
  blk.rp = ds->rp[0] + row_lo;
  blk.col = ds->col[0];
  int32_t *counts, *marg, *dst;
  uint32_t *kept;
  CKR(ar.alloc(&counts, width));
  CKR(ar.alloc(&marg, width));
  CKR(ar.alloc(&kept, U + 1));
  CKR(ar.alloc(&dst, std::max<long long>(blk.nnz, 1)));
  if (m->n_cols > 0) CK(cudaMemcpyAsync(counts, raw_col_counts, sizeof(int32_t) * (size_t)m->n_cols, cudaMemcpyHostToDevice, s));
  CK(cudaMemsetAsync(marg, 0, sizeof(int32_t) * (size_t)width, s));
  CK(cudaMemsetAsync(kept, 0, sizeof(uint32_t) * ((size_t)U + 1), s));
  SampleScratch sc;
  CKR(sample_scratch(c, ar, blk, counts, max_interactions, &sc));
  launch_count(c, blk, sc, max_interactions, seed, flags, nullptr, kept, marg);
  CKR(launch_write(c, ar, blk, sc, dst));
  std::vector<uint32_t> hk((size_t)U + 1);
  CK(cudaMemcpyAsync(hk.data(), kept, sizeof(uint32_t) * hk.size(), cudaMemcpyDeviceToHost, s));
  if (m->n_cols > 0) CK(cudaMemcpyAsync(new_col_counts, marg, sizeof(int32_t) * (size_t)m->n_cols, cudaMemcpyDeviceToHost, s));
  CK(cudaStreamSynchronize(s));
  CK(cudaGetLastError());
  size_t n_kept = 0;
  for (long long r = 0; r < U; ++r) {
    kept_per_row[r] = hk[r];
    if (r >= row_lo && r < row_hi) n_kept += hk[r];
  }
  int32_t *ci = (int32_t *)calloc(std::max<size_t>(n_kept, 1), sizeof(int32_t));
  if (!ci) return set_error(CCO_E_OOM, "malloc failed");
  const size_t n_copy = std::min<size_t>(n_kept, (size_t)blk.nnz);
  if (n_copy) {
    cudaError_t e = cudaMemcpy(ci, dst, sizeof(int32_t) * n_copy, cudaMemcpyDeviceToHost);
    if (e != cudaSuccess) {
      free(ci);
      return set_error(CCO_E_CUDA, "cudaMemcpy: %s", cudaGetErrorString(e));
    }
  }
  *col_idx = ci;
  return CCO_OK;
}

int cco_debug_cooccurrence(cco_ctx_t *c, const cco_csr_t *a, const cco_csr_t *b, int64_t **row_ptr, int32_t **col_idx,
                           int32_t **count) {
  if (!c || !a || !b || !row_ptr || !col_idx || !count) return set_error(CCO_E_INVALID_ARG, "null argument");
  if (c->world != 1 || !c->members.empty()) return set_error(CCO_E_UNSUPPORTED, "debug entries need a single-GPU context");
  cco_csr_t two[2] = {*a, *b};
  cco_indicator_params_t prm[2] = {{0x7fffffff, 1, 0, 0.0}, {0x7fffffff, 1, 0, 0.0}};
  CKR(validate_host(2, two, prm));
  CK(cudaSetDevice(c->device));
  mail_reset(c);
  cudaStream_t s = c->stream;
  cco_dataset *ds = nullptr;
  CKR(dataset_upload(c, 2, two, 0, &ds));
  struct DG { cco_dataset *d; ~DG() { dataset_release(d); } } dg{ds};
  Arena ar(s);
  struct CopyJoin {
    cco_ctx *c;
    ~CopyJoin() { cudaStreamSynchronize(c->copy_stream); }
  } copy_join{c};
  std::vector<DevRaw> raw(2);
  for (int i = 0; i < 2; ++i) {
    raw[i].n_rows = ds->n_users; raw[i].n_cols = (int32_t)ds->n_cols[i]; raw[i].nnz = ds->nnz[i]; raw[i].nnz_cap = ds->nnz[i];
    raw[i].rp = ds->rp[i]; raw[i].col = ds->col[i];
  }
  const std::vector<long long> col_off = {0, raw[0].n_cols, (long long)raw[0].n_cols + raw[1].n_cols};
  const long long width = std::max<long long>(col_off[2], 1);
  int32_t *counts;
  CKR(ar.alloc(&counts, (size_t)width * kHistCopies));
  CK(cudaMemsetAsync(counts, 0, sizeof(int32_t) * (size_t)width * kHistCopies, s));
  CKR(count_raw_columns(c, raw, col_off, ds->ready.data(), nullptr, counts));
  std::vector<DevMat> dm(2);
  for (int i = 0; i < 2; ++i) CKR(downsample_device(c, ar, raw[i], nullptr, counts + col_off[i], 0x7fffffff, 0, 0, &dm[i]));
  const int32_t n_items_a = dm[0].n_cols;
  uint32_t *at_ptr, *cursor, *marg_pad;
  int32_t *at_users, *d_max;
  CKR(ar.alloc(&at_ptr, n_items_a + 1));
  CKR(ar.alloc(&cursor, n_items_a + 1));
  CKR(ar.alloc(&marg_pad, n_items_a + 1));
  CKR(ar.alloc(&d_max, 2));
  CKR(ar.alloc(&at_users, std::max<long long>(raw[0].nnz, 1)));
  CK(cudaMemsetAsync(d_max, 0, 8, s));
  CK(cudaMemcpyAsync(marg_pad, dm[0].marg, sizeof(int32_t) * (size_t)n_items_a, cudaMemcpyDeviceToDevice, s));
  CK(cudaMemsetAsync(marg_pad + n_items_a, 0, 4, s));
  CKR(exclusive_sum(c, ar, marg_pad, at_ptr, (long long)n_items_a + 1));
  CK(cudaMemcpyAsync(cursor, at_ptr, sizeof(uint32_t) * ((size_t)n_items_a + 1), cudaMemcpyDeviceToDevice, s));
  k_transpose_scatter<<<grid_for(a->n_rows * kSG, 256, c->sm_count), 256, 0, s>>>(a->n_rows, dm[0].rp, dm[0].col, cursor, at_users);
  if (n_items_a > 0) k_max_i32<<<grid_for(n_items_a, 256, c->sm_count, 2), 256, 0, s>>>(n_items_a, dm[0].marg, d_max);
  if (dm[1].n_cols > 0) k_max_i32<<<grid_for(dm[1].n_cols, 256, c->sm_count, 2), 256, 0, s>>>(dm[1].n_cols, dm[1].marg, d_max + 1);
  int32_t max_marg_ab[2] = {0, 0};
  CK(cudaMemcpyAsync(max_marg_ab, d_max, 8, cudaMemcpyDeviceToHost, s));
  CK(cudaStreamSynchronize(s));
  CK(cudaGetLastError());
  ResultMat rm;
  IndicatorOut io;
  IndicatorState ist;
  struct EG { IndicatorState &x; ~EG() { if (x.packed) cudaEventDestroy(x.packed); } } eg{ist};
  cco_indicator_params_t p1 = {0x7fffffff, 1, 0, 0.0};
  auto put = [&]() {
    for (void *p : {(void *)rm.row_ptr, (void *)rm.col, (void *)rm.llr, (void *)rm.cnt})
      if (p) c->pinned_put(p);
  };
  int rc = enqueue_indicator(c, ar, at_ptr, at_users, n_items_a, dm[0].marg, max_marg_ab[0], max_marg_ab[1], dm[1], a->n_rows, false, p1,
                             0, true, nullptr, nullptr, nullptr, &ist);
  if (rc == CCO_OK) rc = finish_indicator(c, &ist, 0, 0, &rm, &io);
  cudaStreamSynchronize(c->copy_stream);
  if (rc != CCO_OK) {
    put();
    return rc;
  }
  size_t nnz = (size_t)rm.row_ptr[n_items_a];
  int64_t *rp = (int64_t *)malloc(sizeof(int64_t) * ((size_t)n_items_a + 1));
  int32_t *ci = (int32_t *)malloc(sizeof(int32_t) * std::max<size_t>(nnz, 1));
  int32_t *cn = (int32_t *)malloc(sizeof(int32_t) * std::max<size_t>(nnz, 1));
  if (!rp || !ci || !cn) {
    put();
    return set_error(CCO_E_OOM, "malloc failed");
  }
  memcpy(rp, rm.row_ptr, sizeof(int64_t) * ((size_t)n_items_a + 1));
  std::vector<std::pair<int32_t, int32_t>> tmp;
  for (int32_t r = 0; r < n_items_a; ++r) {
    size_t lo = (size_t)rp[r], hi = (size_t)rp[r + 1];
    tmp.resize(hi - lo);
    for (size_t q = lo; q < hi; ++q) tmp[q - lo] = {rm.col[q], rm.cnt[q]};
    std::sort(tmp.begin(), tmp.end());
    for (size_t q = lo; q < hi; ++q) {
      ci[q] = tmp[q - lo].first;
      cn[q] = tmp[q - lo].second;
    }
  }
  put();
  *row_ptr = rp;
  *col_idx = ci;
  *count = cn;
  return CCO_OK;
}

}
```

### universal_recommender_b200/csrc/cco_kernels.cuh

```cuda
#pragma once

#include <cuda_runtime.h>
#include <stdint.h>

namespace cco {

struct RowArgs {
  const uint32_t *at_ptr;
  const int32_t *at_users;
  const uint32_t *b_ptr;
  const int32_t *b_col;
  const int32_t *marg_a;
  const int32_t *marg_b;
  const int32_t *key_of_col;
  const int32_t *first_key_of_cb;
  int32_t key_shift;
  const uint2 *ext;
  int32_t max_marg_b;
  const int32_t *rows_sorted;
  const uint32_t *row_work;
  const int32_t *bin_bounds;
  int32_t bin;
  int32_t n_cols_b;
  long long n_users;
  int32_t self;
  int32_t top_k;
  int32_t has_min_llr;
  double min_llr;
  int32_t cut_ok;
  double llr_eps2;
  uint32_t flags;
  int32_t count_bits;
  int32_t slots;
  int32_t cap;
  int32_t tsize_x16;
  int32_t cbuf;
  int32_t caux;
  int32_t keep_max;
  int32_t final_max;
  int32_t group_smem_bytes;
  const struct ColTerm *col_terms;
  int32_t out_stride;
  int32_t *out_col;
  double *out_llr;
  int32_t *out_cnt;
  int32_t *out_len;
  unsigned long long *stat_distinct;
  unsigned long long *stat_evaluated;
  int *err_flag;
  int32_t emit_all;
  int32_t bm_words;
};

constexpr uint32_t kEmpty = 0xffffffffu;

__device__ __forceinline__ uint64_t mix64(uint64_t z) {
  z ^= z >> 30;
  z *= 0xbf58476d1ce4e5b9ULL;
  z ^= z >> 27;
  z *= 0x94d049bb133111ebULL;
  z ^= z >> 31;
  return z;
}
__device__ __forceinline__ double sample_u01(int32_t seed, uint32_t u, uint32_t j) {
  uint64_t x = mix64(((uint64_t)(uint32_t)seed << 32) | (uint64_t)u);
  uint64_t h = mix64(x + (uint64_t)j * 0x9e3779b97f4a7c15ULL);
  return __dmul_rn((double)(h >> 11), 0x1.0p-53);
}
__device__ __forceinline__ uint32_t hash32(uint32_t x) {
  x ^= x >> 16;
  x *= 0x7feb352dU;
  x ^= x >> 15;
  x *= 0x846ca68bU;
  x ^= x >> 16;
  return x;
}

__device__ __forceinline__ double xlogx(long long x) {
  return x == 0 ? 0.0 : __dmul_rn((double)x, log((double)x));
}
__device__ __forceinline__ double xlogx_u32(uint32_t x) {
  return x == 0 ? 0.0 : __dmul_rn((double)x, log((double)x));
}
__device__ __forceinline__ double entropy2(long long a, long long b, bool varargs) {
  if (varargs) return __dsub_rn(xlogx(a + b), __dadd_rn(__dadd_rn(0.0, xlogx(a)), xlogx(b)));
  return __dsub_rn(__dsub_rn(xlogx(a + b), xlogx(a)), xlogx(b));
}
__device__ __forceinline__ double entropy4(long long a, long long b, long long c, long long d, bool varargs) {
  if (varargs) {
    double r = __dadd_rn(__dadd_rn(__dadd_rn(__dadd_rn(0.0, xlogx(a)), xlogx(b)), xlogx(c)), xlogx(d));
    return __dsub_rn(xlogx(a + b + c + d), r);
  }
  return __dsub_rn(__dsub_rn(__dsub_rn(__dsub_rn(xlogx(a + b + c + d), xlogx(a)), xlogx(b)), xlogx(c)), xlogx(d));
}
__device__ __forceinline__ double llr_cells(long long k11, long long k12, long long k21, long long k22, bool varargs) {
  double row_e = entropy2(k11 + k12, k21 + k22, varargs);
  double col_e = entropy2(k11 + k21, k12 + k22, varargs);
  double mat_e = entropy4(k11, k12, k21, k22, varargs);
  double s = __dadd_rn(row_e, col_e);
  if (s < mat_e) return 0.0;
  return __dmul_rn(2.0, __dsub_rn(s, mat_e));
}
__device__ __forceinline__ double llr_hoisted(long long k11, long long ra, long long cb, long long n, double row_e,
                                              bool varargs) {
  long long k12 = ra - k11, k21 = cb - k11, k22 = n - ra - cb + k11;
  double col_e = entropy2(cb, n - cb, varargs);
  double mat_e = entropy4(k11, k12, k21, k22, varargs);
  double s = __dadd_rn(row_e, col_e);
  if (s < mat_e) return 0.0;
  return __dmul_rn(2.0, __dsub_rn(s, mat_e));
}

__global__ void k_debug_llr(long long n, const long long *k11, const long long *k12, const long long *k21,
                            const long long *k22, uint32_t flags, double *out) {
  long long i = blockIdx.x * (long long)blockDim.x + threadIdx.x;
  if (i < n) out[i] = llr_cells(k11[i], k12[i], k21[i], k22[i], (flags & CCO_FLAG_ENTROPY_VARARGS) != 0);
}

constexpr int kSG = 8;

constexpr int kHeavyRow = 256;
__global__ void k_list_heavy_rows(long long n_rows, const long long *__restrict__ rp, int32_t *__restrict__ list, int *__restrict__ n_list) {
  for (long long r = blockIdx.x * (long long)blockDim.x + threadIdx.x; r < n_rows; r += (long long)gridDim.x * blockDim.x)
    if (rp[r + 1] - rp[r] > kHeavyRow) list[atomicAdd(n_list, 1)] = (int32_t)r;
}
#define CCO_ROW_LOOP_BEGIN(SG)                                                                         \
  const int lane = threadIdx.x % SG;                                                                   \
  long long it = (blockIdx.x * (long long)blockDim.x + threadIdx.x) / SG;                              \
  const long long stride = (long long)gridDim.x * blockDim.x / SG;                                     \
  const long long n_it = list ? (long long)*n_list : n_rows;                                           \
  for (; it < n_it; it += stride) {                                                                    \
    const long long row = list ? (long long)list[it] : it;
#define CCO_ROW_LOOP_END }

template <int SG>
__global__ void k_check_rows(long long n_rows, int32_t n_cols, const long long *__restrict__ rp, const int32_t *__restrict__ col,
                             long long q_lo, long long q_hi, const int32_t *__restrict__ list, const int *__restrict__ n_list, int *flags) {
  int bad = 0, unsorted = 0;
  CCO_ROW_LOOP_BEGIN(SG)
    long long s = rp[row], e = rp[row + 1];
    if (e < s || s < q_lo || e > q_hi) { bad = 1; continue; }
    if (!list && e - s > kHeavyRow) continue;
    for (long long q = s + lane; q < e; q += SG) {
      int32_t c = col[q];
      if (c < 0 || c >= n_cols) bad = 1;
      if (q > s && col[q - 1] >= c) unsorted = 1;
    }
  CCO_ROW_LOOP_END
  if (bad) atomicOr(&flags[0], 1);
  if (unsorted) atomicOr(&flags[1], 1);
}

__global__ void k_col_histogram(long long row_begin, long long row_end, const long long *__restrict__ rp,
                                const int32_t *__restrict__ col, int32_t n_cols, int32_t *__restrict__ counts, int n_copies,
                                long long copy_stride) {
  const long long s = rp[row_begin], e = rp[row_end];
  const int lane = threadIdx.x & 31;
  int32_t *mine = counts + (long long)(blockIdx.x % n_copies) * copy_stride;
  for (long long q0 = s + blockIdx.x * (long long)blockDim.x + (threadIdx.x & ~31); q0 < e;
       q0 += (long long)gridDim.x * blockDim.x) {
    const long long q = q0 + lane;
    const bool act = q < e;
    const unsigned am = __ballot_sync(0xffffffffu, act);
    if (act) {
      int32_t c = col[q];
      unsigned peers = __match_any_sync(am, c);
      if ((__ffs(peers) - 1) == lane && (uint32_t)c < (uint32_t)n_cols) atomicAdd(&mine[c], __popc(peers));
    }
  }
}
__global__ void k_sum_copies(long long n, int n_copies, long long copy_stride, int32_t *__restrict__ counts) {
  for (long long i = blockIdx.x * (long long)blockDim.x + threadIdx.x; i < n; i += (long long)gridDim.x * blockDim.x) {
    int32_t acc = counts[i];
    for (int k = 1; k < n_copies; ++k) acc += counts[i + k * copy_stride];
    counts[i] = acc;
  }
}

__global__ void k_col_histogram_u32(const uint32_t *__restrict__ lo, const uint32_t *__restrict__ hi,
                                    const int32_t *__restrict__ col, int32_t *__restrict__ counts) {
  const long long s = *lo, e = *hi;
  const int lane = threadIdx.x & 31;
  for (long long q0 = s + blockIdx.x * (long long)blockDim.x + (threadIdx.x & ~31); q0 < e;
       q0 += (long long)gridDim.x * blockDim.x) {
    const long long q = q0 + lane;
    const bool act = q < e;
    const unsigned am = __ballot_sync(0xffffffffu, act);
    if (act) {
      const int32_t c = col[q];
      const unsigned peers = __match_any_sync(am, c);
      if ((__ffs(peers) - 1) == lane) atomicAdd(&counts[c], __popc(peers));
    }
  }
}

__device__ __forceinline__ double row_sample_rate(long long d, int32_t m, bool intdiv) {
  if (d <= 0) return 1.0;
  const long long md = d < m ? d : (long long)m;
  return intdiv ? (double)(md / d) : __ddiv_rn((double)md, (double)d);
}
constexpr unsigned long long kKeepAlways = 1ULL << 53;
__device__ __forceinline__ unsigned long long rate_threshold(double rate) {
  if (rate >= 1.0) return kKeepAlways;
  return (unsigned long long)floor(__dmul_rn(rate, 0x1.0p53));
}
__global__ void k_col_thresholds(int32_t n_cols, const int32_t *__restrict__ raw_counts, int32_t m, unsigned long long *__restrict__ thr) {
  for (int j = blockIdx.x * blockDim.x + threadIdx.x; j < n_cols; j += gridDim.x * blockDim.x) {
    const int32_t c = raw_counts[j];
    thr[j] = c <= m ? kKeepAlways : rate_threshold(__ddiv_rn((double)m, (double)c));
  }
}
__device__ __forceinline__ bool keep_entry_thr(unsigned long long t_row, unsigned long long t_col, uint64_t x_row, uint32_t j) {
  const unsigned long long t = t_row < t_col ? t_row : t_col;
  if (t >= kKeepAlways) return true;
  const uint64_t h = mix64(x_row + (uint64_t)j * 0x9e3779b97f4a7c15ULL);
  return (h >> 11) <= t;
}

template <int SG>
__global__ void k_downsample_count(long long n_rows, long long row_base, const long long *__restrict__ rp, const int32_t *__restrict__ col,
                                   int32_t n_cols, long long q_lo, long long q_hi, const unsigned long long *__restrict__ col_thr, int32_t m,
                                   int32_t seed, uint32_t flags, const int32_t *__restrict__ list, const int *__restrict__ n_list,
                                   uint32_t *__restrict__ kept_per_row, int32_t *__restrict__ new_counts, uint8_t *__restrict__ keep_flag) {
  const unsigned sg_mask = SG == 32 ? 0xffffffffu : (((1u << SG) - 1u) << ((threadIdx.x & 31) / SG * SG));
  const bool intdiv = (flags & CCO_FLAG_ROWRATE_INTDIV) != 0;
  CCO_ROW_LOOP_BEGIN(SG)
    long long s = rp[row], e = rp[row + 1], d = e - s;
    if (!list && d > kHeavyRow) continue;
    if (d < 0 || s < q_lo || e > q_hi) continue;
    const unsigned long long t_row = rate_threshold(row_sample_rate(d, m, intdiv));
    const uint32_t g = (uint32_t)(row_base + row);
    const uint64_t x_row = mix64(((uint64_t)(uint32_t)seed << 32) | (uint64_t)g);
    uint32_t kept = 0;
    for (long long q0 = s; q0 < e; q0 += SG) {
      long long q = q0 + lane;
      bool keep = false;
      int32_t j = 0;
      if (q < e) {
        j = col[q];
        keep = (uint32_t)j < (uint32_t)n_cols && keep_entry_thr(t_row, col_thr[j], x_row, (uint32_t)j);
        keep_flag[q - q_lo] = keep ? 1 : 0;
      }
      if (keep && new_counts) atomicAdd(&new_counts[j], 1);
      kept += __popc(__ballot_sync(sg_mask, keep) & sg_mask);
    }
    if (lane == 0) kept_per_row[g] = kept;
  CCO_ROW_LOOP_END
}

template <int SG>
__global__ void k_downsample_write(long long n_rows, long long row_base, const long long *__restrict__ rp, const int32_t *__restrict__ col,
                                   long long q_lo, long long q_hi, const uint8_t *__restrict__ keep_flag,
                                   const int32_t *__restrict__ list, const int *__restrict__ n_list,
                                   const uint32_t *__restrict__ new_ptr, const uint32_t *__restrict__ out_base, int32_t *__restrict__ new_col) {
  const int sg_shift = SG == 32 ? 0 : (threadIdx.x & 31) / SG * SG;
  const unsigned sg_mask = SG == 32 ? 0xffffffffu : (((1u << SG) - 1u) << sg_shift);
  const uint32_t base = out_base ? *out_base : 0u;
  CCO_ROW_LOOP_BEGIN(SG)
    long long s = rp[row], e = rp[row + 1], d = e - s;
    if (!list && d > kHeavyRow) continue;
    if (d < 0 || s < q_lo || e > q_hi) continue;
    uint32_t w = new_ptr[row_base + row] - base;
    for (long long q0 = s; q0 < e; q0 += SG) {
      long long q = q0 + lane;
      bool keep = false;
      int32_t j = 0;
      if (q < e) {
        j = col[q];
        keep = keep_flag[q - q_lo] != 0;
      }
      unsigned b = (__ballot_sync(sg_mask, keep) & sg_mask) >> sg_shift;
      if (keep) new_col[w + __popc(b & ((1u << lane) - 1u))] = j;
      w += __popc(b);
    }
  CCO_ROW_LOOP_END
}

__global__ void k_pack_blocks(int world, long long S, long long U, long long cap, const uint32_t *__restrict__ new_ptr,
                              const int32_t *__restrict__ gathered, int32_t *__restrict__ new_col) {
  for (int q = blockIdx.y; q < world; q += gridDim.y) {
    const long long u0 = min((long long)q * S, U), u1 = min(u0 + S, U);
    const uint32_t lo = new_ptr[u0], hi = new_ptr[u1];
    const int32_t *src = gathered + (long long)q * cap;
    for (uint32_t i = blockIdx.x * blockDim.x + threadIdx.x; i < hi - lo; i += gridDim.x * blockDim.x) new_col[lo + i] = src[i];
  }
}

__global__ void k_transpose_scatter(long long n_rows, const uint32_t *__restrict__ rp, const int32_t *__restrict__ col,
                                    uint32_t *__restrict__ cursor, int32_t *__restrict__ users) {
  const int lane = threadIdx.x % kSG;
  long long row = (blockIdx.x * (long long)blockDim.x + threadIdx.x) / kSG;
  const long long stride = (long long)gridDim.x * blockDim.x / kSG;
  for (; row < n_rows; row += stride) {
    uint32_t s = rp[row], e = rp[row + 1];
    for (uint32_t q = s + lane; q < e; q += kSG) users[atomicAdd(&cursor[col[q]], 1u)] = (int32_t)row;
  }
}

__global__ void k_row_work(int32_t n_items, const uint32_t *__restrict__ at_ptr, const int32_t *__restrict__ at_users,
                           const uint32_t *__restrict__ b_ptr, uint32_t *__restrict__ row_work,
                           unsigned long long *__restrict__ work64, int32_t *__restrict__ item_ids,
                           uint2 *__restrict__ ext) {
  const int lane = threadIdx.x % kSG;
  const unsigned sg_mask = ((1u << kSG) - 1u) << ((threadIdx.x & 31) / kSG * kSG);
  int item = (blockIdx.x * blockDim.x + threadIdx.x) / kSG;
  const int stride = gridDim.x * blockDim.x / kSG;
  for (; item < n_items; item += stride) {
    uint32_t s = at_ptr[item], e = at_ptr[item + 1];
    unsigned long long w = 0;
    for (uint32_t q = s + lane; q < e; q += kSG) {
      int32_t u = at_users[q];
      const uint32_t bs = b_ptr[u], bl = b_ptr[u + 1] - bs;
      w += bl;
      if (ext) ext[q] = make_uint2(bs, bl);
    }
#pragma unroll
    for (int o = kSG / 2; o > 0; o >>= 1) w += __shfl_xor_sync(sg_mask, w, o);
    if (lane == 0) {
      row_work[item] = w > 0xffffffffULL ? 0xffffffffu : (uint32_t)w;
      work64[item] = w;
      item_ids[item] = item;
    }
  }
}

struct BinThresholds {
  uint32_t t[12];
};
__global__ void k_bin_bounds(int32_t n_rows, const uint32_t *__restrict__ sorted_work, int32_t n_bins,
                             const BinThresholds thresholds, int32_t *__restrict__ bounds) {
  int b = threadIdx.x;
  if (b > n_bins) return;
  if (b == 0) { bounds[0] = 0; return; }
  uint32_t t = b == n_bins ? 0u : thresholds.t[b - 1];
  int lo = 0, hi = n_rows;
  while (lo < hi) {
    int mid = (lo + hi) >> 1;
    if (sorted_work[mid] > t) lo = mid + 1; else hi = mid;
  }
  bounds[b] = lo;
}

struct __align__(16) ColTerm {
  double col_e;
  double x_cbm1;
  int32_t cb;
  int32_t col;
  int32_t pad[2];
};
__global__ void k_col_terms(int32_t n_cols, const int32_t *__restrict__ marg_key, const int32_t *__restrict__ col_of_key,
                            long long n_users, uint32_t flags, ColTerm *__restrict__ out) {
  const bool varargs = (flags & CCO_FLAG_ENTROPY_VARARGS) != 0;
  for (int i = blockIdx.x * blockDim.x + threadIdx.x; i < n_cols; i += gridDim.x * blockDim.x) {
    long long cb = marg_key[i];
    ColTerm t;
    t.col_e = entropy2(cb, n_users - cb, varargs);
    t.x_cbm1 = cb >= 1 ? xlogx(cb - 1) : 0.0;
    t.cb = (int32_t)cb;
    t.col = col_of_key[i];
    t.pad[0] = t.pad[1] = 0;
    out[i] = t;
  }
}

__global__ void k_col_order_init(int32_t n_cols, const int32_t *__restrict__ marg, uint32_t *__restrict__ cb_out,
                                 int32_t *__restrict__ id_out) {
  for (int i = blockIdx.x * blockDim.x + threadIdx.x; i < n_cols; i += gridDim.x * blockDim.x) {
    cb_out[i] = (uint32_t)marg[i];
    id_out[i] = i;
  }
}
__global__ void k_col_order(int32_t n_cols, int32_t max_cb, const uint32_t *__restrict__ marg_key, const int32_t *__restrict__ col_of_key,
                            int32_t *__restrict__ key_of_col, int32_t *__restrict__ first_key_of_cb) {
  for (int k = blockIdx.x * blockDim.x + threadIdx.x; k < n_cols; k += gridDim.x * blockDim.x) {
    key_of_col[col_of_key[k]] = k;
    const int32_t cb = (int32_t)marg_key[k], lo = k == 0 ? 0 : (int32_t)marg_key[k - 1] + 1;
    for (int32_t c = lo; c <= cb; ++c) first_key_of_cb[c] = k;
    if (k == n_cols - 1)
      for (int32_t c = cb + 1; c <= max_cb + 1; ++c) first_key_of_cb[c] = n_cols;
  }
}
__global__ void k_relabel_cols(const uint32_t *__restrict__ end, const int32_t *__restrict__ key_of_col, int32_t *__restrict__ col) {
  const long long n = *end;
  for (long long q = blockIdx.x * (long long)blockDim.x + threadIdx.x; q < n; q += (long long)gridDim.x * blockDim.x)
    col[q] = key_of_col[col[q]];
}

__device__ __forceinline__ bool cand_better(const uint4 &p, const uint4 &q) {
  return p.y > q.y || (p.y == q.y && (p.x > q.x || (p.x == q.x && p.z < q.z)));
}

template <int GROUP>
__device__ __forceinline__ void group_sync() {
  if (GROUP == 32) __syncwarp(); else __syncthreads();
}

template <int GROUP>
__device__ void sort_candidates(uint4 *tk, int n, int gtid) {
  int n2 = 1;
  while (n2 < n) n2 <<= 1;
  for (int i = n + gtid; i < n2; i += GROUP) tk[i] = make_uint4(0u, 0u, 0xffffffffu, 0u);
  group_sync<GROUP>();
  for (int k2 = 2; k2 <= n2; k2 <<= 1) {
    for (int j = k2 >> 1; j > 0; j >>= 1) {
      for (int t = gtid; t < (n2 >> 1); t += GROUP) {
        const int i = ((t & ~(j - 1)) << 1) | (t & (j - 1));
        const int p = i | j;
        const bool up = (i & k2) == 0;
        const uint4 ei = tk[i], ep = tk[p];
        const bool swap = up ? cand_better(ep, ei) : cand_better(ei, ep);
        if (swap) { tk[i] = ep; tk[p] = ei; }
      }
      group_sync<GROUP>();
    }
  }
}

__device__ __forceinline__ uint32_t cand_word(const uint4 &e, int wi) { return wi == 0 ? e.y : (wi == 1 ? e.x : ~e.z); }

template <int GROUP>
__device__ int reduce_candidates(uint4 *tk, uint4 *aux, int n, int k, int M, int *hist, int *ctrl, int gtid) {
  volatile int *vc = ctrl;
  uint32_t pre0 = 0u, pre1 = 0u, pre2 = 0u;
  int nb = 0, above = 0, kept = n;
  while (true) {
    for (int i = gtid; i < 256; i += GROUP) hist[i] = 0;
    group_sync<GROUP>();
    const int wi = nb >> 5, sh = 24 - (nb & 31);
    for (int i = gtid; i < n; i += GROUP) {
      const uint4 e = tk[i];
      const uint32_t w0 = e.y, w1 = e.x, w2 = ~e.z;
      bool match;
      if (nb == 0) match = true;
      else if (nb < 32) match = (w0 >> (32 - nb)) == (pre0 >> (32 - nb));
      else if (nb == 32) match = w0 == pre0;
      else if (nb < 64) match = w0 == pre0 && (w1 >> (64 - nb)) == (pre1 >> (64 - nb));
      else if (nb == 64) match = w0 == pre0 && w1 == pre1;
      else match = w0 == pre0 && w1 == pre1 && (w2 >> (96 - nb)) == (pre2 >> (96 - nb));
      if (match) atomicAdd(&hist[__byte_perm(cand_word(e, wi), 0u, 0x4440u | (uint32_t)(sh >> 3))], 1);
    }
    group_sync<GROUP>();
    if (gtid < 32) {
      int c[8], ssum = 0;
#pragma unroll
      for (int j = 0; j < 8; ++j) { c[j] = hist[255 - 8 * gtid - j]; ssum += c[j]; }
      int incl = ssum;
#pragma unroll
      for (int d = 1; d < 32; d <<= 1) {
        const int v = __shfl_up_sync(0xffffffffu, incl, d);
        if (gtid >= d) incl += v;
      }
      const int excl = incl - ssum, need = k - above;
      if (excl < need && need <= incl) {
        int run = excl;
#pragma unroll
        for (int j = 0; j < 8; ++j) {
          if (run < need && run + c[j] >= need) { ctrl[24] = 255 - 8 * gtid - j; ctrl[25] = run; ctrl[26] = c[j]; }
          run += c[j];
        }
      }
    }
    group_sync<GROUP>();
    const int D = vc[24], c_gt = vc[25], c_d = vc[26];
    if (wi == 0) pre0 |= (uint32_t)D << sh; else if (wi == 1) pre1 |= (uint32_t)D << sh; else pre2 |= (uint32_t)D << sh;
    nb += 8;
    kept = above + c_gt + c_d;
    if (kept <= M || nb == 96) break;
    above += c_gt;
    group_sync<GROUP>();
  }
  if (gtid == 0) ctrl[27] = 0;
  group_sync<GROUP>();
  if (GROUP == 32) {
    int w = 0;
    for (int i0 = 0; i0 < n; i0 += 32) {
      const int i = i0 + gtid;
      uint4 e = make_uint4(0u, 0u, 0u, 0u);
      bool keep = false;
      if (i < n) {
        e = tk[i];
        const uint32_t w0 = e.y, w1 = e.x, w2 = ~e.z;
        keep = w0 > pre0 || (w0 == pre0 && (w1 > pre1 || (w1 == pre1 && w2 >= pre2)));
      }
      const unsigned m = __ballot_sync(0xffffffffu, keep);
      __syncwarp();
      if (keep) tk[w + __popc(m & ((1u << gtid) - 1u))] = e;
      w += __popc(m);
      __syncwarp();
    }
  } else {
    for (int i = gtid; i < n; i += GROUP) {
      const uint4 e = tk[i];
      const uint32_t w0 = e.y, w1 = e.x, w2 = ~e.z;
      const bool keep = w0 > pre0 || (w0 == pre0 && (w1 > pre1 || (w1 == pre1 && w2 >= pre2)));
      if (keep) aux[atomicAdd(&ctrl[27], 1)] = e;
    }
    group_sync<GROUP>();
    for (int i = gtid; i < kept; i += GROUP) tk[i] = aux[i];
  }
  if (gtid == 0) {
    ctrl[0] = kept;
    ctrl[4] = (int)pre1; ctrl[5] = (int)pre0; ctrl[6] = (int)~pre2; ctrl[7] = 0;
    ctrl[1] = 1;
  }
  group_sync<GROUP>();
  return kept;
}

constexpr int kCutBins = 512;
constexpr int kDomLevels = 15;
constexpr int kX12N = 31;

__device__ __forceinline__ void cut_find(const uint32_t *h1, uint32_t need, int lane, int *ctrl) {
  uint32_t sum = 0;
  for (int wi = 0; wi < 8; ++wi) { const uint32_t v = h1[lane * 8 + wi]; sum += (v & 0xffffu) + (v >> 16); }
  uint32_t incl = sum;
#pragma unroll
  for (int d = 1; d < 32; d <<= 1) {
    const uint32_t v = __shfl_up_sync(0xffffffffu, incl, d);
    if (lane >= d) incl += v;
  }
  const uint32_t excl = incl - sum;
  int found = 0x7fffffff;
  uint32_t below = 0;
  if (excl < need && incl >= need) {
    uint32_t run = excl;
    for (int wi = 0; wi < 8; ++wi) {
      const uint32_t v = h1[lane * 8 + wi];
      if (run + (v & 0xffffu) >= need) { found = lane * 16 + 2 * wi; below = run; break; }
      run += v & 0xffffu;
      if (run + (v >> 16) >= need) { found = lane * 16 + 2 * wi + 1; below = run; break; }
      run += v >> 16;
    }
  }
#pragma unroll
  for (int o = 16; o > 0; o >>= 1) {
    found = min(found, __shfl_xor_sync(0xffffffffu, found, o));
    below = max(below, __shfl_xor_sync(0xffffffffu, below, o));
  }
  if (lane == 0) { ctrl[9] = found; ctrl[10] = (int)below; }
}

template <int GROUP, bool DENSE>
__device__ __forceinline__ void accumulate(uint32_t *table, uint32_t tsize, uint32_t b, int cbits, uint32_t n_pass,
                                           uint32_t pass, int *err_flag) {
  if (DENSE) {
    atomicAdd(&table[b], 1u);
    return;
  }
  if (n_pass > 1 && ((b * 0x85ebca6bu) >> 12) % n_pass != pass) return;
  uint32_t slot = __umulhi(b * 0x9e3779b1u, tsize);
  const uint32_t want = b << cbits;
  uint32_t probes = 0;
  while (true) {
    const uint32_t w = *reinterpret_cast<volatile uint32_t *>(&table[slot]);
    if ((w >> cbits) == b && w != kEmpty) { atomicAdd(&table[slot], 1u); return; }
    if (w == kEmpty) {
      const uint32_t old = atomicCAS(&table[slot], kEmpty, want | 1u);
      if (old == kEmpty) return;
      if ((old >> cbits) == b) { atomicAdd(&table[slot], 1u); return; }
    }
    slot = (slot + 1 == tsize) ? 0 : slot + 1;
    if (++probes > tsize) { atomicOr(err_flag, 1); return; }
  }
}

template <int GROUP, bool DENSE, bool BITMAP>
__device__ __forceinline__ void count_window(const RowArgs &a, uint32_t *table, uint32_t *seen, uint32_t tsize, int cbits,
                                             uint32_t n_pass, uint32_t pass, uint32_t off, uint32_t s, uint32_t p_lo,
                                             uint32_t p_hi, int lane) {
  for (uint32_t p0 = p_lo; p0 < p_hi; p0 += 64) {
    uint32_t bb[2];
    bool act[2];
#pragma unroll
    for (int h = 0; h < 2; ++h) {
      const uint32_t p = p0 + h * 32 + lane;
      int j = 0;
#pragma unroll
      for (int st = 16; st > 0; st >>= 1) {
        const int c = j + st;
        const uint32_t v = __shfl_sync(0xffffffffu, off, c);
        if (v <= p) j = c;
      }
      const uint32_t sj = __shfl_sync(0xffffffffu, s, j), oj = __shfl_sync(0xffffffffu, off, j);
      act[h] = p < p_hi;
      bb[h] = act[h] ? (uint32_t)a.b_col[sj + (p - oj)] : 0u;
    }
    if (BITMAP) {
      uint32_t old[2];
#pragma unroll
      for (int h = 0; h < 2; ++h) old[h] = act[h] ? atomicOr(&seen[bb[h] >> 5], 1u << (bb[h] & 31u)) : 0u;
#pragma unroll
      for (int h = 0; h < 2; ++h)
        if (act[h] && ((old[h] >> (bb[h] & 31u)) & 1u)) accumulate<GROUP, false>(table, tsize, bb[h], cbits, 1u, 0u, a.err_flag);
    } else {
#pragma unroll
      for (int h = 0; h < 2; ++h)
        if (act[h]) accumulate<GROUP, DENSE>(table, tsize, bb[h], cbits, n_pass, pass, a.err_flag);
// ... 576 lines not shown
```

### universal_recommender_b200/csrc/cco_sampler.cuh

```cuda
#pragma once

#include <cuda_runtime.h>
#include <stdint.h>

#include "cco_kernels.cuh"

namespace cco {

constexpr int kSampleChunk = 256;

__device__ __forceinline__ long long warp_find_row(const long long *__restrict__ rp, long long n_rows, long long q, int lane) {
  long long lo = 0, hi = n_rows;
  while (hi - lo > 1) {
    const long long step = (hi - lo + 31) / 32;
    const long long p = lo + lane * step;
    const bool ok = p < hi && rp[p] <= q;
    const unsigned b = __ballot_sync(0xffffffffu, ok) | 1u;
    const int top = 31 - __clz(b);
    lo += top * step;
    hi = hi < lo + step ? hi : lo + step;
  }
  return lo;
}

__global__ void __launch_bounds__(256) k_sample_count(long long n_rows, long long row_base, const long long *__restrict__ rp,
                                                      const int32_t *__restrict__ col, int32_t n_cols, long long q_lo, long long q_hi,
                                                      const unsigned long long *__restrict__ col_thr, int32_t m, int32_t seed, uint32_t flags,
                                                      const int *__restrict__ bad ,
                                                      uint32_t *__restrict__ kept_per_row , int32_t *__restrict__ new_counts,
                                                      uint8_t *__restrict__ keep_flag) {
  const int lane = threadIdx.x & 31;
  const long long warp = (blockIdx.x * (long long)blockDim.x + threadIdx.x) >> 5;
  const long long n_warps = ((long long)gridDim.x * blockDim.x) >> 5;
  const long long n_chunks = (q_hi - q_lo + kSampleChunk - 1) / kSampleChunk;
  const bool intdiv = (flags & CCO_FLAG_ROWRATE_INTDIV) != 0;
  const long long kNoRow = 0x7fffffffffffffffLL;
  if (n_rows <= 0) return;
  if (bad && *bad) {
    for (long long q = blockIdx.x * (long long)blockDim.x + threadIdx.x; q < q_hi - q_lo; q += (long long)gridDim.x * blockDim.x) keep_flag[q] = 0;
    return;
  }
  for (long long chunk = warp; chunk < n_chunks; chunk += n_warps) {
    const long long Q0 = q_lo + chunk * kSampleChunk;
    const long long Q1 = Q0 + kSampleChunk < q_hi ? Q0 + kSampleChunk : q_hi;
    long long base = warp_find_row(rp, n_rows, Q0, lane);
    long long start_i, end_i;
    unsigned long long t_i, x_i;
    uint32_t kept_i;
#define CCO_LOAD_WINDOW()                                                                                   \
  {                                                                                                         \
    const long long r = base + lane;                                                                        \
    start_i = end_i = kNoRow;                                                                               \
    t_i = kKeepAlways;                                                                                      \
    x_i = 0;                                                                                                \
    if (r < n_rows) {                                                                                       \
      start_i = rp[r];                                                                                      \
      end_i = rp[r + 1];                                                                                    \
      const long long d = end_i - start_i;                                                                  \
      if (d > (long long)m) t_i = rate_threshold(row_sample_rate(d, m, intdiv));  \
      x_i = mix64(((uint64_t)(uint32_t)seed << 32) | (uint64_t)(uint32_t)(row_base + r));                   \
    }                                                                                                       \
    kept_i = 0;                                                                                             \
  }
#define CCO_FLUSH_WINDOW()                                                                                  \
  if (kept_i) atomicAdd(&kept_per_row[row_base + base + lane], kept_i);
    CCO_LOAD_WINDOW()
    for (long long qb = Q0; qb < Q1; qb += 32) {
      const long long q = qb + lane;
      bool pending = q < Q1;
      const int32_t j = pending ? col[q] : 0;
      unsigned long long t_col = kKeepAlways;
      if (pending && (uint32_t)j < (uint32_t)n_cols) t_col = col_thr[j];
      while (true) {
        int idx = 0;
#pragma unroll
        for (int step = 16; step > 0; step >>= 1) {
          const long long v = __shfl_sync(0xffffffffu, end_i, idx + step - 1);
          if (v <= q) idx += step;
        }
        {
          const long long v = __shfl_sync(0xffffffffu, end_i, idx);
          if (v <= q) idx += 1;
        }
        const int src = idx & 31;
        const unsigned long long t_row = __shfl_sync(0xffffffffu, t_i, src);
        const unsigned long long x_row = __shfl_sync(0xffffffffu, x_i, src);
        const bool here = pending && idx < 32;
        const bool real_row = base + idx < n_rows;
        bool keep = false;
        if (here) {
          keep = real_row && (uint32_t)j < (uint32_t)n_cols && keep_entry_thr(t_row, t_col, x_row, (uint32_t)j);
          keep_flag[q - q_lo] = keep ? 1 : 0;
          if (keep && new_counts) atomicAdd(&new_counts[j], 1);
        }
        const unsigned kb = __ballot_sync(0xffffffffu, keep);
        const int a = start_i <= qb ? 0 : (start_i >= qb + 32 ? 32 : (int)(start_i - qb));
        const int b = end_i <= qb ? 0 : (end_i >= qb + 32 ? 32 : (int)(end_i - qb));
        if (b > a) {
          const unsigned below_b = b >= 32 ? 0xffffffffu : ((1u << b) - 1u);
          const unsigned below_a = (1u << a) - 1u;
          kept_i += __popc(kb & below_b & ~below_a);
        }
        pending = pending && !here;
        if (!__any_sync(0xffffffffu, pending)) break;
        CCO_FLUSH_WINDOW()
        base += 32;
        if (base >= n_rows) {
          if (pending) keep_flag[q - q_lo] = 0;
          kept_i = 0;
          start_i = end_i = kNoRow;
          break;
        }
        CCO_LOAD_WINDOW()
      }
      if (base >= n_rows) {
        for (long long q2 = qb + 32 + lane; q2 < Q1; q2 += 32) keep_flag[q2 - q_lo] = 0;
        break;
      }
    }
    if (base < n_rows && base + lane < n_rows) { CCO_FLUSH_WINDOW() }
#undef CCO_LOAD_WINDOW
#undef CCO_FLUSH_WINDOW
  }
}

__global__ void k_check_row_ptr(long long n_rows, const long long *__restrict__ rp, long long q_lo, long long q_hi, int *flags) {
  int bad = 0;
  for (long long r = blockIdx.x * (long long)blockDim.x + threadIdx.x; r < n_rows; r += (long long)gridDim.x * blockDim.x) {
    const long long s = rp[r], e = rp[r + 1];
    if (e < s || s < q_lo || e > q_hi) bad = 1;
  }
  if (bad) atomicOr(&flags[0], 1);
}
template <bool AGG>
__global__ void k_col_histogram_flat(long long n, const int32_t *__restrict__ col, int32_t n_cols, int32_t *__restrict__ counts, int n_copies,
                                     long long copy_stride, int *flags ) {
  int32_t *mine = counts + (long long)(blockIdx.x % n_copies) * copy_stride;
  const int lane = threadIdx.x & 31;
  int bad = 0;
  for (long long q0 = blockIdx.x * (long long)blockDim.x + (threadIdx.x & ~31); q0 < n; q0 += (long long)gridDim.x * blockDim.x) {
    const long long q = q0 + lane;
    const bool act = q < n;
    const int32_t j = act ? col[q] : -1;
    const bool ok = act && (uint32_t)j < (uint32_t)n_cols;
    if (act && !ok) bad = 1;
    if (AGG) {
      const unsigned om = __ballot_sync(0xffffffffu, ok);
      if (ok) {
        const unsigned peers = __match_any_sync(om, j);
        if ((__ffs(peers) - 1) == lane) atomicAdd(&mine[j], __popc(peers));
      }
    } else if (ok) {
      atomicAdd(&mine[j], 1);
    }
  }
  if (flags && bad) atomicOr(&flags[0], 1);
}

}
```

Baseline: 4.152 billion.

## Batch per-matrix sampling into grouped kernels with bitmask keep flags and chunk scan

```diff
diff --git a/universal_recommender_b200/csrc/cco_api.cu b/universal_recommender_b200/csrc/cco_api.cu
--- a/universal_recommender_b200/csrc/cco_api.cu
+++ b/universal_recommender_b200/csrc/cco_api.cu
@@ -476,90 +476,121 @@
   k_check_rows<32><<<c->sm_count * 4, 256, 0, c->stream>>>(raw.n_rows, raw.n_cols, raw.rp, raw.col, q_lo, q_hi, h.list, h.n, flags);
   c->launches += 2;
 }
-struct SampleScratch {
-  unsigned long long *col_thr = nullptr;
-  uint8_t *keep = nullptr;
+struct PrepGroup {
+  PrepMats d;
+  int first = 0;
+  long long chunk0 = 0, rows = 0, cols = 0;
 };
-static int sample_scratch(cco_ctx *c, Arena &ar, const DevRaw &raw, const int32_t *raw_counts, int32_t m, SampleScratch *sc) {
-  CKR(ar.alloc(&sc->col_thr, std::max<int32_t>(raw.n_cols, 1)));
-  CKR(ar.alloc(&sc->keep, std::max<long long>(raw.nnz, 1)));
-  if (raw.n_cols > 0) {
-    k_col_thresholds<<<grid_for(raw.n_cols, 256, c->sm_count, 4), 256, 0, c->stream>>>(raw.n_cols, raw_counts, m, sc->col_thr);
-    c->launches++;
-  }
-  return CCO_OK;
-}
-static void launch_count(cco_ctx *c, const DevRaw &raw, const SampleScratch &sc, int32_t m, int32_t seed, uint32_t flags, const int *bad,
-                         uint32_t *kept, int32_t *new_counts) {
-  if (raw.n_rows <= 0 || raw.nnz <= 0) return;
-  const long long q_lo = raw.q_base, q_hi = raw.q_base + raw.nnz;
-  const long long n_chunks = (raw.nnz + kSampleChunk - 1) / kSampleChunk;
-  k_sample_count<<<grid_for(n_chunks * 32, 256, c->sm_count), 256, 0, c->stream>>>(raw.n_rows, raw.row_base, raw.rp, raw.col, raw.n_cols, q_lo, q_hi,
-                                                                                  sc.col_thr, m, seed, flags, bad, kept, new_counts, sc.keep);
-  c->launches++;
-}
-static int launch_write(cco_ctx *c, Arena &ar, const DevRaw &raw, const SampleScratch &sc, int32_t *dst) {
-  if (raw.n_rows <= 0 || raw.nnz <= 0) return CCO_OK;
-  long long *n_sel;
-  CKR(ar.alloc(&n_sel, 1));
-  size_t tb = 0;
-  CK(cub::DeviceSelect::Flagged(nullptr, tb, raw.col + raw.q_base, sc.keep, dst, n_sel, (long long)raw.nnz, c->stream));
-  void *tmp;
-  CKR(ar.alloc((char **)&tmp, tb));
-  CK(cub::DeviceSelect::Flagged(tmp, tb, raw.col + raw.q_base, sc.keep, dst, n_sel, (long long)raw.nnz, c->stream));
-  ar.release(tmp);
-  c->launches += 2;
-  return CCO_OK;
-}
-
-constexpr int kHistCopies = 16;
+static std::vector<PrepGroup> prep_groups(const std::vector<DevRaw> &raw) {
+  std::vector<PrepGroup> gs;
+  long long chunk = 0;
+  for (int i = 0; i < (int)raw.size(); ++i) {
+    if (i % kPrepMats == 0) {
+      gs.emplace_back();
+      gs.back().first = i;
+      gs.back().chunk0 = chunk;
+    }
+    PrepGroup &g = gs.back();
+    PrepMats &d = g.d;
+    const int k = d.n++;
+    PrepMat &M = d.mat[k];
+    M.n_rows = raw[i].n_rows;
+    M.row_base = raw[i].row_base;
+    M.q_lo = raw[i].q_base;
+    M.q_hi = raw[i].q_base + raw[i].nnz;
+    M.rp = raw[i].rp;
+    M.col = raw[i].col;
+    M.n_cols = raw[i].n_cols;
+    const long long n_chunks = (raw[i].nnz + kSampleChunk - 1) / kSampleChunk;
+    d.chunk_off[k + 1] = d.chunk_off[k] + n_chunks;
+    d.row_off[k + 1] = d.row_off[k] + raw[i].n_rows;
+    d.col_off[k + 1] = d.col_off[k] + raw[i].n_cols;
+    g.rows = d.row_off[k + 1];
+    g.cols = d.col_off[k + 1];
+    chunk += n_chunks;
+  }
+  return gs;
+}
+static long long prep_chunks(const std::vector<PrepGroup> &gs) {
+  return gs.empty() ? 0 : gs.back().chunk0 + gs.back().d.chunk_off[gs.back().d.n];
+}
+
 static int count_raw_columns(cco_ctx *c, const std::vector<DevRaw> &raw, const std::vector<long long> &col_off, const cudaEvent_t *ready,
                              int *verdict, int32_t *counts) {
   cudaStream_t s = c->stream;
   const int n_mats = (int)raw.size();
-  const long long total_cols = col_off[n_mats];
-  const long long copy_stride = std::max<long long>(total_cols, 1);
-  for (int i = 0; i < n_mats; ++i) {
-    if (ready) CK(cudaStreamWaitEvent(s, ready[i], 0));
-    if (raw[i].n_rows == 0) continue;
-    int *v = verdict ? verdict + 2 * i : nullptr;
-    if (v) {
-      k_check_row_ptr<<<grid_for(raw[i].n_rows, 256, c->sm_count), 256, 0, s>>>(raw[i].n_rows, raw[i].rp, raw[i].q_base, raw[i].q_base + raw[i].nnz, v);
+  if (ready)
+    for (int i = 0; i < n_mats; ++i) CK(cudaStreamWaitEvent(s, ready[i], 0));
+  std::vector<PrepGroup> gs = prep_groups(raw);
+  for (PrepGroup &g : gs) {
+    for (int k = 0; k < g.d.n; ++k) {
+      const int i = g.first + k;
+      g.d.mat[k].counts = counts + col_off[i];
+      g.d.mat[k].bad = verdict ? verdict + 2 * i : nullptr;
+    }
+    const long long work = std::max(g.rows, g.d.chunk_off[g.d.n] * kSampleChunk);
+    if (work == 0) continue;
+    k_raw_counts<<<grid_for(work, kSampleChunk, c->sm_count, 7), kSampleChunk, 0, s>>>(g.d);
+    c->launches++;
+  }
+  return CCO_OK;
+}
+
+struct SampleState {
+  std::vector<PrepGroup> gs;
+  unsigned long long *col_thr = nullptr;
+  uint32_t *keep = nullptr;
+  long long *chunk_kept = nullptr, *chunk_pos = nullptr;
+};
+static int sample_pass1(cco_ctx *c, Arena &ar, const std::vector<DevRaw> &raw, const int32_t *raw_counts, const std::vector<long long> &col_off,
+                        const std::vector<int32_t> &m, int32_t seed, uint32_t flags, int *verdict, const std::vector<uint32_t *> &kept,
+                        const std::vector<int32_t *> &marg, SampleState *st) {
+  cudaStream_t s = c->stream;
+  st->gs = prep_groups(raw);
+  const long long n_chunks = prep_chunks(st->gs);
+  CKR(ar.alloc(&st->col_thr, std::max<long long>(col_off[raw.size()], 1)));
+  CKR(ar.alloc(&st->keep, std::max<long long>(n_chunks * kChunkWords, 1)));
+  CKR(ar.alloc(&st->chunk_kept, n_chunks + 1));
+  CKR(ar.alloc(&st->chunk_pos, n_chunks + 1));
+  CK(cudaMemsetAsync(st->chunk_kept + n_chunks, 0, sizeof(long long), s));
+  for (PrepGroup &g : st->gs) {
+    for (int k = 0; k < g.d.n; ++k) {
+      const int i = g.first + k;
+      PrepMat &M = g.d.mat[k];
+      M.m = m[i];
+      M.bad = verdict ? verdict + 2 * i : nullptr;
+      M.col_thr = st->col_thr + col_off[i];
+      M.keep = st->keep + (g.chunk0 + g.d.chunk_off[k]) * kChunkWords;
+      M.kept_per_row = kept[i];
+      M.counts = const_cast<int32_t *>(raw_counts) + col_off[i];
+    }
+    if (g.cols > 0) {
+      k_col_thresholds<<<grid_for(g.cols, 256, c->sm_count, 4), 256, 0, s>>>(g.d);
       c->launches++;
     }
-    if (raw[i].nnz > 0) {
-      k_col_histogram_flat<true><<<grid_for(raw[i].nnz, 256, c->sm_count), 256, 0, s>>>(raw[i].nnz, raw[i].col + raw[i].q_base, raw[i].n_cols,
-                                                                                       counts + col_off[i], kHistCopies, copy_stride, v);
+    for (int k = 0; k < g.d.n; ++k) g.d.mat[k].counts = marg[g.first + k];
+    const long long g_chunks = g.d.chunk_off[g.d.n];
+    if (g_chunks > 0) {
+      k_sample_keep<<<grid_for(g_chunks * 32, 256, c->sm_count), 256, 0, s>>>(g.d, seed, flags, st->chunk_kept + g.chunk0);
       c->launches++;
     }
   }
-  if (total_cols > 0) {
-    k_sum_copies<<<grid_for(total_cols, 256, c->sm_count), 256, 0, s>>>(total_cols, kHistCopies, copy_stride, counts);
-    c->launches++;
-  }
-  return CCO_OK;
-}
-
-static int downsample_device(cco_ctx *c, Arena &ar, const DevRaw &raw, const int *bad, const int32_t *raw_counts, int32_t m,
-                             int32_t seed, uint32_t flags, DevMat *out) {
-  out->n_rows = raw.n_rows;
-  out->n_cols = raw.n_cols;
-  uint32_t *kept;
-  CKR(ar.alloc(&kept, raw.n_rows + 1));
-  CKR(ar.alloc(&out->rp, raw.n_rows + 1));
-  if (!out->marg) CKR(ar.alloc(&out->marg, std::max<int32_t>(raw.n_cols, 1)));
-  CKR(ar.alloc(&out->col, std::max<long long>(raw.nnz, 1)));
-  CK(cudaMemsetAsync(out->marg, 0, sizeof(int32_t) * std::max<int32_t>(raw.n_cols, 1), c->stream));
-  CK(cudaMemsetAsync(kept, 0, sizeof(uint32_t) * ((size_t)raw.n_rows + 1), c->stream));
-  SampleScratch sc;
-  CKR(sample_scratch(c, ar, raw, raw_counts, m, &sc));
-  launch_count(c, raw, sc, m, seed, flags, bad, kept, out->marg);
-  CKR(exclusive_sum(c, ar, kept, out->rp, raw.n_rows + 1));
-  CKR(launch_write(c, ar, raw, sc, out->col));
+  return exclusive_sum(c, ar, st->chunk_kept, st->chunk_pos, n_chunks + 1);
+}
+static int sample_pass2(cco_ctx *c, Arena &ar, SampleState *st, const std::vector<int32_t *> &dst) {
+  for (PrepGroup &g : st->gs) {
+    for (int k = 0; k < g.d.n; ++k) g.d.mat[k].dst = dst[g.first + k];
+    const long long g_chunks = g.d.chunk_off[g.d.n];
+    if (g_chunks > 0) {
+      k_sample_write<<<grid_for(g_chunks * 32, 256, c->sm_count), 256, 0, c->stream>>>(g.d, st->chunk_pos + g.chunk0);
+      c->launches++;
+    }
+  }
   CK(cudaGetLastError());
-  ar.release(kept);
-  ar.release(sc.col_thr);
-  ar.release(sc.keep);
+  ar.release(st->col_thr);
+  ar.release(st->keep);
+  ar.release(st->chunk_kept);
+  ar.release(st->chunk_pos);
   return CCO_OK;
 }
 
@@ -568,72 +599,84 @@
   return CCO_OK;
 }
 
-static int downsample_sharded_all(cco_ctx *c, Arena &ar, const std::vector<DevRaw> &raw, const int *d_check ,
-                                  const std::vector<long long> &block_cap,
-                                  long long U, const int32_t *raw_counts, int32_t *marg_all, const std::vector<long long> &col_off,
-                                  const cco_indicator_params_t *params, int32_t seed, uint32_t flags, std::vector<DevMat> &dm,
-                                  cudaEvent_t *stage_ev ) {
+static int downsample_all(cco_ctx *c, Arena &ar, const std::vector<DevRaw> &raw, int *d_check ,
+                          long long U, const int32_t *raw_counts, int32_t *marg_all, const std::vector<long long> &col_off,
+                          const cco_indicator_params_t *params, int32_t seed, uint32_t flags, std::vector<DevMat> &dm,
+                          cudaEvent_t *stage_ev ) {
   cudaStream_t s = c->stream;
   const int W = c->world, r = c->rank, n_mats = (int)raw.size();
   const long long S = (U + W - 1) / W;
-  const long long row_base = raw[0].row_base;
+  const long long kept_len = W * S + 1;
+  uint32_t *kept_all;
+  CKR(ar.alloc(&kept_all, std::max<long long>((long long)n_mats * kept_len, 1)));
+  CK(cudaMemsetAsync(kept_all, 0, sizeof(uint32_t) * (size_t)n_mats * (size_t)kept_len, s));
   std::vector<uint32_t *> kept(n_mats, nullptr);
-  std::vector<SampleScratch> sc(n_mats);
+  std::vector<int32_t *> marg(n_mats, nullptr);
+  std::vector<int32_t> m(n_mats);
   for (int i = 0; i < n_mats; ++i) {
     DevMat *out = &dm[i];
     out->n_rows = U;
     out->n_cols = raw[i].n_cols;
-    out->marg = marg_all + col_off[i];
-    CKR(ar.alloc(&kept[i], (size_t)(W * S + 1)));
+    out->marg = marg[i] = marg_all + col_off[i];
+    kept[i] = kept_all + (size_t)i * kept_len;
+    m[i] = params[i].max_interactions;
     CKR(ar.alloc(&out->rp, U + 1));
-    CK(cudaMemsetAsync(kept[i], 0, sizeof(uint32_t) * (size_t)(W * S + 1), s));
-    CKR(sample_scratch(c, ar, raw[i], raw_counts + col_off[i], params[i].max_interactions, &sc[i]));
-    launch_count(c, raw[i], sc[i], params[i].max_interactions, seed, flags, d_check + 2 * i, kept[i], out->marg);
-  }
+  }
+  SampleState st;
+  CKR(sample_pass1(c, ar, raw, raw_counts, col_off, m, seed, flags, d_check, kept, marg, &st));
   CK(cudaEventRecord(stage_ev[0], s));
-  if (S > 0) {
-    g_nccl.GroupStart();
-    for (int i = 0; i < n_mats; ++i) {
-      int rc = g_nccl.AllGather(kept[i] + (size_t)r * S, kept[i], (size_t)S, kNcclUint32, c->comm, s);
-      if (rc != 0) { g_nccl.GroupEnd(); return nccl_check(rc, "ncclAllGather(kept counts)"); }
-    }
-    CKR(nccl_check(g_nccl.GroupEnd(), "ncclGroupEnd(kept counts)"));
-  }
-  if (col_off[n_mats] > 0)
-    CKR(nccl_check(g_nccl.AllReduce(marg_all, marg_all, (size_t)col_off[n_mats], kNcclInt32, kNcclSum, c->comm, s), "ncclAllReduce(marginals)"));
-  std::vector<int32_t *> gathered(n_mats, nullptr);
+  if (W > 1) {
+    if (S > 0) {
+      g_nccl.GroupStart();
+      for (int i = 0; i < n_mats; ++i) {
+        int rc = g_nccl.AllGather(kept[i] + (size_t)r * S, kept[i], (size_t)S, kNcclUint32, c->comm, s);
+        if (rc != 0) { g_nccl.GroupEnd(); return nccl_check(rc, "ncclAllGather(kept counts)"); }
+      }
+      CKR(nccl_check(g_nccl.GroupEnd(), "ncclGroupEnd(kept counts)"));
+    }
+    if (col_off[n_mats] > 0)
+      CKR(nccl_check(g_nccl.AllReduce(marg_all, marg_all, (size_t)col_off[n_mats], kNcclInt32, kNcclSum, c->comm, s), "ncclAllReduce(marginals)"));
+  }
   std::vector<uint32_t> edge((size_t)n_mats * (W + 1), 0);
   for (int i = 0; i < n_mats; ++i) {
     CKR(exclusive_sum(c, ar, kept[i], dm[i].rp, U + 1));
-    ar.release(kept[i]);
-    for (int q = 0; q <= W; ++q) CKR(mail_fetch(c, &edge[(size_t)i * (W + 1) + q], dm[i].rp + std::min<long long>((long long)q * S, U), 4));
-  }
+    if (W > 1)
+      for (int q = 0; q <= W; ++q) CKR(mail_fetch(c, &edge[(size_t)i * (W + 1) + q], dm[i].rp + std::min<long long>((long long)q * S, U), 4));
+  }
+  ar.release(kept_all);
   CK(cudaEventRecord(stage_ev[1], s));
-  CKR(mail_wait(c));
   std::vector<long long> cap(n_mats, 0);
+  std::vector<int32_t *> gathered(n_mats, nullptr), dst(n_mats, nullptr);
+  if (W > 1) CKR(mail_wait(c));
   for (int i = 0; i < n_mats; ++i) {
+    if (W == 1) {
+      CKR(ar.alloc(&dm[i].col, std::max<long long>(raw[i].nnz, 1)));
+      dst[i] = dm[i].col;
+      continue;
+    }
     for (int q = 0; q < W; ++q) cap[i] = std::max<long long>(cap[i], (long long)edge[(size_t)i * (W + 1) + q + 1] - edge[(size_t)i * (W + 1) + q]);
     CKR(ar.alloc(&dm[i].col, std::max<long long>(edge[(size_t)i * (W + 1) + W], 1)));
     if (cap[i] == 0) continue;
     CKR(ar.alloc(&gathered[i], (size_t)(cap[i] * W)));
-    CKR(launch_write(c, ar, raw[i], sc[i], gathered[i] + (size_t)r * cap[i]));
-    ar.release(sc[i].col_thr);
-    ar.release(sc[i].keep);
-  }
+    dst[i] = gathered[i] + (size_t)r * cap[i];
+  }
+  CKR(sample_pass2(c, ar, &st, dst));
   CK(cudaEventRecord(stage_ev[2], s));
-  g_nccl.GroupStart();
-  for (int i = 0; i < n_mats; ++i) {
-    if (!gathered[i]) continue;
-    int rc = g_nccl.AllGather(gathered[i] + (size_t)r * cap[i], gathered[i], (size_t)cap[i], kNcclInt32, c->comm, s);
-    if (rc != 0) { g_nccl.GroupEnd(); return nccl_check(rc, "ncclAllGather(column blocks)"); }
-  }
-  CKR(nccl_check(g_nccl.GroupEnd(), "ncclGroupEnd(column blocks)"));
-  for (int i = 0; i < n_mats; ++i) {
-    if (!gathered[i]) continue;
-    dim3 grid((unsigned)std::max(1, std::min(c->sm_count * 8 / W, 1024)), (unsigned)W);
-    k_pack_blocks<<<grid, 256, 0, s>>>(W, S, U, cap[i], dm[i].rp, gathered[i], dm[i].col);
-    c->launches++;
-    ar.release(gathered[i]);
+  if (W > 1) {
+    g_nccl.GroupStart();
+    for (int i = 0; i < n_mats; ++i) {
+      if (!gathered[i]) continue;
+      int rc = g_nccl.AllGather(gathered[i] + (size_t)r * cap[i], gathered[i], (size_t)cap[i], kNcclInt32, c->comm, s);
+      if (rc != 0) { g_nccl.GroupEnd(); return nccl_check(rc, "ncclAllGather(column blocks)"); }
+    }
+    CKR(nccl_check(g_nccl.GroupEnd(), "ncclGroupEnd(column blocks)"));
+    for (int i = 0; i < n_mats; ++i) {
+      if (!gathered[i]) continue;
+      dim3 grid((unsigned)std::max(1, std::min(c->sm_count * 8 / W, 1024)), (unsigned)W);
+      k_pack_blocks<<<grid, 256, 0, s>>>(W, S, U, cap[i], dm[i].rp, gathered[i], dm[i].col);
+      c->launches++;
+      ar.release(gathered[i]);
+    }
   }
   CK(cudaEventRecord(stage_ev[3], s));
   CK(cudaGetLastError());
@@ -1297,14 +1340,14 @@
     total_cols += raw[i].n_cols;
   }
   col_off[n_mats] = total_cols;
-  const long long copy_stride = std::max<long long>(total_cols, 1);
+  const long long n_counts = std::max<long long>(total_cols, 1);
   int32_t *raw_counts, *marg_all;
   int *d_check;
-  CKR(ar.alloc(&raw_counts, (size_t)copy_stride * kHistCopies));
-  CKR(ar.alloc(&marg_all, (size_t)copy_stride));
+  CKR(ar.alloc(&raw_counts, (size_t)n_counts));
+  CKR(ar.alloc(&marg_all, (size_t)n_counts));
   CKR(ar.alloc(&d_check, 2 * n_mats));
-  CK(cudaMemsetAsync(raw_counts, 0, sizeof(int32_t) * (size_t)copy_stride * kHistCopies, s));
-  CK(cudaMemsetAsync(marg_all, 0, sizeof(int32_t) * (size_t)copy_stride, s));
+  CK(cudaMemsetAsync(raw_counts, 0, sizeof(int32_t) * (size_t)n_counts, s));
+  CK(cudaMemsetAsync(marg_all, 0, sizeof(int32_t) * (size_t)n_counts, s));
   CK(cudaMemsetAsync(d_check, 0, sizeof(int) * 2 * n_mats, s));
   CKR(count_raw_columns(c, raw, col_off, ds->ready.data(), ds->validated ? nullptr : d_check, raw_counts));
   CK(mark(0));
@@ -1315,18 +1358,7 @@
   }
   CK(mark(1));
   std::vector<DevMat> dm(n_mats);
-  if (c->world > 1) {
-    CKR(downsample_sharded_all(c, ar, raw, d_check, ds->block_cap, n_users, raw_counts, marg_all, col_off, params, seed, flags, dm, &sev[2]));
-  } else {
-    for (int i = 0; i < n_mats; ++i) {
-      dm[i].marg = marg_all + col_off[i];
-      CKR(downsample_device(c, ar, raw[i], d_check + 2 * i, raw_counts + col_off[i], params[i].max_interactions, seed, flags, &dm[i]));
-    }
-    CK(mark(2));
-    CK(mark(3));
-    CK(mark(4));
-    CK(mark(5));
-  }
+  CKR(downsample_all(c, ar, raw, d_check, n_users, raw_counts, marg_all, col_off, params, seed, flags, dm, &sev[2]));
   const int32_t n_items_a = dm[0].n_cols;
   uint32_t *at_ptr, *cursor;
   int32_t *at_users, *d_max;
@@ -1344,7 +1376,8 @@
     ar.release(marg_pad);
   }
   CK(cudaMemcpyAsync(cursor, at_ptr, sizeof(uint32_t) * ((size_t)n_items_a + 1), cudaMemcpyDeviceToDevice, s));
-  k_transpose_scatter<<<grid_for(n_users * kSG, 256, c->sm_count), 256, 0, s>>>(n_users, dm[0].rp, dm[0].col, cursor, at_users);
+  k_transpose_scatter<<<grid_for((ds->nnz[0] + kSampleChunk - 1) / kSampleChunk * 32, 256, c->sm_count), 256, 0, s>>>(n_users, dm[0].rp, dm[0].col,
+                                                                                                                   cursor, at_users);
   c->launches++;
   for (int i = 0; i < n_mats; ++i)
     if (dm[i].n_cols > 0) {
@@ -4492,14 +4525,21 @@
   const int32_t width = std::max<int32_t>(m->n_cols, 1);
   int32_t *counts;
   int *d_check;
-  CKR(ar.alloc(&counts, (size_t)width * kHistCopies));
+  CKR(ar.alloc(&counts, (size_t)width));
   CKR(ar.alloc(&d_check, 2));
-  CK(cudaMemsetAsync(counts, 0, sizeof(int32_t) * (size_t)width * kHistCopies, c->stream));
+  CK(cudaMemsetAsync(counts, 0, sizeof(int32_t) * (size_t)width, c->stream));
   CK(cudaMemsetAsync(d_check, 0, sizeof(int) * 2, c->stream));
   int *verdict = ds->validated ? nullptr : d_check;
   CKR(count_raw_columns(c, raw, col_off, ds->ready.data(), verdict, counts));
-  DevMat dm;
-  CKR(downsample_device(c, ar, raw[0], verdict, counts, max_interactions, seed, flags, &dm));
+  std::vector<DevMat> dms(1);
+  int32_t *marg;
+  CKR(ar.alloc(&marg, width));
+  CK(cudaMemsetAsync(marg, 0, sizeof(int32_t) * (size_t)width, c->stream));
+  cudaEvent_t stage_ev[4];
+  c->ev_timing_used = c->ev_plain_used = 0;
+  for (auto &e : stage_ev) CKR(pooled_event(c, false, &e));
+  CKR(downsample_all(c, ar, raw, verdict, raw[0].n_rows, counts, marg, col_off, &prm, seed, flags, dms, stage_ev));
+  const DevMat &dm = dms[0];
   std::vector<uint32_t> rp32((size_t)m->n_rows + 1);
   int h_check = 0;
   CK(cudaMemcpyAsync(rp32.data(), dm.rp, sizeof(uint32_t) * rp32.size(), cudaMemcpyDeviceToHost, c->stream));
@@ -4564,10 +4604,10 @@
   if (m->n_cols > 0) CK(cudaMemcpyAsync(counts, raw_col_counts, sizeof(int32_t) * (size_t)m->n_cols, cudaMemcpyHostToDevice, s));
   CK(cudaMemsetAsync(marg, 0, sizeof(int32_t) * (size_t)width, s));
   CK(cudaMemsetAsync(kept, 0, sizeof(uint32_t) * ((size_t)U + 1), s));
-  SampleScratch sc;
-  CKR(sample_scratch(c, ar, blk, counts, max_interactions, &sc));
-  launch_count(c, blk, sc, max_interactions, seed, flags, nullptr, kept, marg);
-  CKR(launch_write(c, ar, blk, sc, dst));
+  SampleState sst;
+  const std::vector<DevRaw> blks = {blk};
+  CKR(sample_pass1(c, ar, blks, counts, {0, m->n_cols}, {max_interactions}, seed, flags, nullptr, {kept}, {marg}, &sst));
+  CKR(sample_pass2(c, ar, &sst, {dst}));
   std::vector<uint32_t> hk((size_t)U + 1);
   CK(cudaMemcpyAsync(hk.data(), kept, sizeof(uint32_t) * hk.size(), cudaMemcpyDeviceToHost, s));
   if (m->n_cols > 0) CK(cudaMemcpyAsync(new_col_counts, marg, sizeof(int32_t) * (size_t)m->n_cols, cudaMemcpyDeviceToHost, s));
@@ -4618,11 +4658,17 @@
   const std::vector<long long> col_off = {0, raw[0].n_cols, (long long)raw[0].n_cols + raw[1].n_cols};
   const long long width = std::max<long long>(col_off[2], 1);
   int32_t *counts;
-  CKR(ar.alloc(&counts, (size_t)width * kHistCopies));
-  CK(cudaMemsetAsync(counts, 0, sizeof(int32_t) * (size_t)width * kHistCopies, s));
+  CKR(ar.alloc(&counts, (size_t)width));
+  CK(cudaMemsetAsync(counts, 0, sizeof(int32_t) * (size_t)width, s));
   CKR(count_raw_columns(c, raw, col_off, ds->ready.data(), nullptr, counts));
   std::vector<DevMat> dm(2);
-  for (int i = 0; i < 2; ++i) CKR(downsample_device(c, ar, raw[i], nullptr, counts + col_off[i], 0x7fffffff, 0, 0, &dm[i]));
+  int32_t *marg;
+  CKR(ar.alloc(&marg, width));
+  CK(cudaMemsetAsync(marg, 0, sizeof(int32_t) * (size_t)width, s));
+  cudaEvent_t stage_ev[4];
+  c->ev_timing_used = c->ev_plain_used = 0;
+  for (auto &e : stage_ev) CKR(pooled_event(c, false, &e));
+  CKR(downsample_all(c, ar, raw, nullptr, ds->n_users, counts, marg, col_off, prm, 0, 0, dm, stage_ev));
   const int32_t n_items_a = dm[0].n_cols;
   uint32_t *at_ptr, *cursor, *marg_pad;
   int32_t *at_users, *d_max;
@@ -4636,7 +4682,8 @@
   CK(cudaMemsetAsync(marg_pad + n_items_a, 0, 4, s));
   CKR(exclusive_sum(c, ar, marg_pad, at_ptr, (long long)n_items_a + 1));
   CK(cudaMemcpyAsync(cursor, at_ptr, sizeof(uint32_t) * ((size_t)n_items_a + 1), cudaMemcpyDeviceToDevice, s));
-  k_transpose_scatter<<<grid_for(a->n_rows * kSG, 256, c->sm_count), 256, 0, s>>>(a->n_rows, dm[0].rp, dm[0].col, cursor, at_users);
+  k_transpose_scatter<<<grid_for((raw[0].nnz + kSampleChunk - 1) / kSampleChunk * 32, 256, c->sm_count), 256, 0, s>>>(a->n_rows, dm[0].rp, dm[0].col,
+                                                                                                                 cursor, at_users);
   if (n_items_a > 0) k_max_i32<<<grid_for(n_items_a, 256, c->sm_count, 2), 256, 0, s>>>(n_items_a, dm[0].marg, d_max);
   if (dm[1].n_cols > 0) k_max_i32<<<grid_for(dm[1].n_cols, 256, c->sm_count, 2), 256, 0, s>>>(dm[1].n_cols, dm[1].marg, d_max + 1);
   int32_t max_marg_ab[2] = {0, 0};
diff --git a/universal_recommender_b200/csrc/cco_kernels.cuh b/universal_recommender_b200/csrc/cco_kernels.cuh
--- a/universal_recommender_b200/csrc/cco_kernels.cuh
+++ b/universal_recommender_b200/csrc/cco_kernels.cuh
@@ -151,32 +151,6 @@
   if (unsorted) atomicOr(&flags[1], 1);
 }
 
-__global__ void k_col_histogram(long long row_begin, long long row_end, const long long *__restrict__ rp,
-                                const int32_t *__restrict__ col, int32_t n_cols, int32_t *__restrict__ counts, int n_copies,
-                                long long copy_stride) {
-  const long long s = rp[row_begin], e = rp[row_end];
-  const int lane = threadIdx.x & 31;
-  int32_t *mine = counts + (long long)(blockIdx.x % n_copies) * copy_stride;
-  for (long long q0 = s + blockIdx.x * (long long)blockDim.x + (threadIdx.x & ~31); q0 < e;
-       q0 += (long long)gridDim.x * blockDim.x) {
-    const long long q = q0 + lane;
-    const bool act = q < e;
-    const unsigned am = __ballot_sync(0xffffffffu, act);
-    if (act) {
-      int32_t c = col[q];
-      unsigned peers = __match_any_sync(am, c);
-      if ((__ffs(peers) - 1) == lane && (uint32_t)c < (uint32_t)n_cols) atomicAdd(&mine[c], __popc(peers));
-    }
-  }
-}
-__global__ void k_sum_copies(long long n, int n_copies, long long copy_stride, int32_t *__restrict__ counts) {
-  for (long long i = blockIdx.x * (long long)blockDim.x + threadIdx.x; i < n; i += (long long)gridDim.x * blockDim.x) {
-    int32_t acc = counts[i];
-    for (int k = 1; k < n_copies; ++k) acc += counts[i + k * copy_stride];
-    counts[i] = acc;
-  }
-}
-
 __global__ void k_col_histogram_u32(const uint32_t *__restrict__ lo, const uint32_t *__restrict__ hi,
                                     const int32_t *__restrict__ col, int32_t *__restrict__ counts) {
   const long long s = *lo, e = *hi;
@@ -204,76 +178,11 @@
   if (rate >= 1.0) return kKeepAlways;
   return (unsigned long long)floor(__dmul_rn(rate, 0x1.0p53));
 }
-__global__ void k_col_thresholds(int32_t n_cols, const int32_t *__restrict__ raw_counts, int32_t m, unsigned long long *__restrict__ thr) {
-  for (int j = blockIdx.x * blockDim.x + threadIdx.x; j < n_cols; j += gridDim.x * blockDim.x) {
-    const int32_t c = raw_counts[j];
-    thr[j] = c <= m ? kKeepAlways : rate_threshold(__ddiv_rn((double)m, (double)c));
-  }
-}
 __device__ __forceinline__ bool keep_entry_thr(unsigned long long t_row, unsigned long long t_col, uint64_t x_row, uint32_t j) {
   const unsigned long long t = t_row < t_col ? t_row : t_col;
   if (t >= kKeepAlways) return true;
   const uint64_t h = mix64(x_row + (uint64_t)j * 0x9e3779b97f4a7c15ULL);
   return (h >> 11) <= t;
-}
-
-template <int SG>
-__global__ void k_downsample_count(long long n_rows, long long row_base, const long long *__restrict__ rp, const int32_t *__restrict__ col,
-                                   int32_t n_cols, long long q_lo, long long q_hi, const unsigned long long *__restrict__ col_thr, int32_t m,
-                                   int32_t seed, uint32_t flags, const int32_t *__restrict__ list, const int *__restrict__ n_list,
-                                   uint32_t *__restrict__ kept_per_row, int32_t *__restrict__ new_counts, uint8_t *__restrict__ keep_flag) {
-  const unsigned sg_mask = SG == 32 ? 0xffffffffu : (((1u << SG) - 1u) << ((threadIdx.x & 31) / SG * SG));
-  const bool intdiv = (flags & CCO_FLAG_ROWRATE_INTDIV) != 0;
-  CCO_ROW_LOOP_BEGIN(SG)
-    long long s = rp[row], e = rp[row + 1], d = e - s;
-    if (!list && d > kHeavyRow) continue;
-    if (d < 0 || s < q_lo || e > q_hi) continue;
-    const unsigned long long t_row = rate_threshold(row_sample_rate(d, m, intdiv));
-    const uint32_t g = (uint32_t)(row_base + row);
-    const uint64_t x_row = mix64(((uint64_t)(uint32_t)seed << 32) | (uint64_t)g);
-    uint32_t kept = 0;
-    for (long long q0 = s; q0 < e; q0 += SG) {
-      long long q = q0 + lane;
-      bool keep = false;
-      int32_t j = 0;
-      if (q < e) {
-        j = col[q];
-        keep = (uint32_t)j < (uint32_t)n_cols && keep_entry_thr(t_row, col_thr[j], x_row, (uint32_t)j);
-        keep_flag[q - q_lo] = keep ? 1 : 0;
-      }
-      if (keep && new_counts) atomicAdd(&new_counts[j], 1);
-      kept += __popc(__ballot_sync(sg_mask, keep) & sg_mask);
-    }
-    if (lane == 0) kept_per_row[g] = kept;
-  CCO_ROW_LOOP_END
-}
-
-template <int SG>
-__global__ void k_downsample_write(long long n_rows, long long row_base, const long long *__restrict__ rp, const int32_t *__restrict__ col,
-                                   long long q_lo, long long q_hi, const uint8_t *__restrict__ keep_flag,
-                                   const int32_t *__restrict__ list, const int *__restrict__ n_list,
-                                   const uint32_t *__restrict__ new_ptr, const uint32_t *__restrict__ out_base, int32_t *__restrict__ new_col) {
-  const int sg_shift = SG == 32 ? 0 : (threadIdx.x & 31) / SG * SG;
-  const unsigned sg_mask = SG == 32 ? 0xffffffffu : (((1u << SG) - 1u) << sg_shift);
-  const uint32_t base = out_base ? *out_base : 0u;
-  CCO_ROW_LOOP_BEGIN(SG)
-    long long s = rp[row], e = rp[row + 1], d = e - s;
-    if (!list && d > kHeavyRow) continue;
-    if (d < 0 || s < q_lo || e > q_hi) continue;
-    uint32_t w = new_ptr[row_base + row] - base;
-    for (long long q0 = s; q0 < e; q0 += SG) {
-      long long q = q0 + lane;
-      bool keep = false;
-      int32_t j = 0;
-      if (q < e) {
-        j = col[q];
-        keep = keep_flag[q - q_lo] != 0;
-      }
-      unsigned b = (__ballot_sync(sg_mask, keep) & sg_mask) >> sg_shift;
-      if (keep) new_col[w + __popc(b & ((1u << lane) - 1u))] = j;
-      w += __popc(b);
-    }
-  CCO_ROW_LOOP_END
 }
 
 __global__ void k_pack_blocks(int world, long long S, long long U, long long cap, const uint32_t *__restrict__ new_ptr,
@@ -283,17 +192,6 @@
     const uint32_t lo = new_ptr[u0], hi = new_ptr[u1];
     const int32_t *src = gathered + (long long)q * cap;
     for (uint32_t i = blockIdx.x * blockDim.x + threadIdx.x; i < hi - lo; i += gridDim.x * blockDim.x) new_col[lo + i] = src[i];
-  }
-}
-
-__global__ void k_transpose_scatter(long long n_rows, const uint32_t *__restrict__ rp, const int32_t *__restrict__ col,
-                                    uint32_t *__restrict__ cursor, int32_t *__restrict__ users) {
-  const int lane = threadIdx.x % kSG;
-  long long row = (blockIdx.x * (long long)blockDim.x + threadIdx.x) / kSG;
-  const long long stride = (long long)gridDim.x * blockDim.x / kSG;
-  for (; row < n_rows; row += stride) {
-    uint32_t s = rp[row], e = rp[row + 1];
-    for (uint32_t q = s + lane; q < e; q += kSG) users[atomicAdd(&cursor[col[q]], 1u)] = (int32_t)row;
   }
 }
 
diff --git a/universal_recommender_b200/csrc/cco_sampler.cuh b/universal_recommender_b200/csrc/cco_sampler.cuh
--- a/universal_recommender_b200/csrc/cco_sampler.cuh
+++ b/universal_recommender_b200/csrc/cco_sampler.cuh
@@ -8,13 +8,41 @@
 namespace cco {
 
 constexpr int kSampleChunk = 256;
-
-__device__ __forceinline__ long long warp_find_row(const long long *__restrict__ rp, long long n_rows, long long q, int lane) {
+constexpr int kChunkWords = kSampleChunk / 32;
+constexpr int kPrepMats = 16;
+
+struct PrepMat {
+  long long n_rows = 0, row_base = 0, q_lo = 0, q_hi = 0;
+  const long long *rp = nullptr;
+  const int32_t *col = nullptr;
+  int32_t n_cols = 0, m = 0;
+  int32_t *counts = nullptr;
+  int *bad = nullptr;
+  unsigned long long *col_thr = nullptr;
+  uint32_t *kept_per_row = nullptr;
+  uint32_t *keep = nullptr;
+  int32_t *dst = nullptr;
+};
+struct PrepMats {
+  int n = 0;
+  long long chunk_off[kPrepMats + 1] = {};
+  long long row_off[kPrepMats + 1] = {};
+  long long col_off[kPrepMats + 1] = {};
+  PrepMat mat[kPrepMats];
+};
+__device__ __forceinline__ int prep_mat_of(const long long *off, int n, long long x) {
+  int i = 0;
+  while (i + 1 < n && x >= off[i + 1]) ++i;
+  return i;
+}
+
+template <typename P>
+__device__ __forceinline__ long long warp_find_row(const P *__restrict__ rp, long long n_rows, long long q, int lane) {
   long long lo = 0, hi = n_rows;
   while (hi - lo > 1) {
     const long long step = (hi - lo + 31) / 32;
     const long long p = lo + lane * step;
-    const bool ok = p < hi && rp[p] <= q;
+    const bool ok = p < hi && (long long)rp[p] <= q;
     const unsigned b = __ballot_sync(0xffffffffu, ok) | 1u;
     const int top = 31 - __clz(b);
     lo += top * step;
@@ -23,27 +51,96 @@
   return lo;
 }
 
-__global__ void __launch_bounds__(256) k_sample_count(long long n_rows, long long row_base, const long long *__restrict__ rp,
-                                                      const int32_t *__restrict__ col, int32_t n_cols, long long q_lo, long long q_hi,
-                                                      const unsigned long long *__restrict__ col_thr, int32_t m, int32_t seed, uint32_t flags,
-                                                      const int *__restrict__ bad ,
-                                                      uint32_t *__restrict__ kept_per_row , int32_t *__restrict__ new_counts,
-                                                      uint8_t *__restrict__ keep_flag) {
+constexpr int kHotSlots = 4096;
+__device__ __forceinline__ void flush_hot(int32_t *hot_col, uint32_t *hot_n, int32_t *counts) {
+  for (int s = threadIdx.x; s < kHotSlots; s += blockDim.x) {
+    if (hot_n[s]) atomicAdd(&counts[hot_col[s]], (int32_t)hot_n[s]);
+    hot_n[s] = 0;
+    hot_col[s] = -1;
+  }
+}
+__global__ void __launch_bounds__(kSampleChunk) k_raw_counts(const __grid_constant__ PrepMats d) {
+  __shared__ int32_t hot_col[kHotSlots];
+  __shared__ uint32_t hot_n[kHotSlots];
+  const long long tid = blockIdx.x * (long long)blockDim.x + threadIdx.x, nthr = (long long)gridDim.x * blockDim.x;
+  int i = 0;
+  for (long long r = tid; r < d.row_off[d.n]; r += nthr) {
+    while (r >= d.row_off[i + 1]) ++i;
+    const PrepMat &M = d.mat[i];
+    if (!M.bad) continue;
+    const long long k = r - d.row_off[i];
+    const long long s = M.rp[k], e = M.rp[k + 1];
+    if (e < s || s < M.q_lo || e > M.q_hi) atomicOr(M.bad, 1);
+  }
+  for (int s = threadIdx.x; s < kHotSlots; s += blockDim.x) {
+    hot_col[s] = -1;
+    hot_n[s] = 0;
+  }
+  int cur = -1;
+  for (long long g = blockIdx.x; g < d.chunk_off[d.n]; g += gridDim.x) {
+    i = prep_mat_of(d.chunk_off, d.n, g);
+    if (i != cur) {
+      __syncthreads();
+      if (cur >= 0) flush_hot(hot_col, hot_n, d.mat[cur].counts);
+      cur = i;
+      __syncthreads();
+    }
+    const PrepMat &M = d.mat[i];
+    const long long q = M.q_lo + (g - d.chunk_off[i]) * kSampleChunk + threadIdx.x;
+    if (q >= M.q_hi) continue;
+    const int32_t j = M.col[q];
+    if ((uint32_t)j >= (uint32_t)M.n_cols) {
+      if (M.bad) atomicOr(M.bad, 1);
+      continue;
+    }
+    const int s = (int)(((uint32_t)j * 0x9E3779B1u) >> 20);
+    int k = ((volatile int32_t *)hot_col)[s];
+    if (k == -1) {
+      k = atomicCAS(&hot_col[s], -1, j);
+      if (k == -1) k = j;
+    }
+    if (k == j) atomicAdd(&hot_n[s], 1u);
+    else atomicAdd(&M.counts[j], 1);
+  }
+  __syncthreads();
+  if (cur >= 0) flush_hot(hot_col, hot_n, d.mat[cur].counts);
+}
+
+__global__ void k_col_thresholds(const __grid_constant__ PrepMats d) {
+  const long long tid = blockIdx.x * (long long)blockDim.x + threadIdx.x, nthr = (long long)gridDim.x * blockDim.x;
+  int i = 0;
+  for (long long x = tid; x < d.col_off[d.n]; x += nthr) {
+    while (x >= d.col_off[i + 1]) ++i;
+    const PrepMat &M = d.mat[i];
+    const long long j = x - d.col_off[i];
+    const int32_t c = M.counts[j];
+    M.col_thr[j] = c <= M.m ? kKeepAlways : rate_threshold(__ddiv_rn((double)M.m, (double)c));
+  }
+}
+
+__global__ void __launch_bounds__(256) k_sample_keep(const __grid_constant__ PrepMats d, int32_t seed, uint32_t flags,
+                                                     long long *__restrict__ chunk_kept) {
   const int lane = threadIdx.x & 31;
   const long long warp = (blockIdx.x * (long long)blockDim.x + threadIdx.x) >> 5;
   const long long n_warps = ((long long)gridDim.x * blockDim.x) >> 5;
-  const long long n_chunks = (q_hi - q_lo + kSampleChunk - 1) / kSampleChunk;
   const bool intdiv = (flags & CCO_FLAG_ROWRATE_INTDIV) != 0;
   const long long kNoRow = 0x7fffffffffffffffLL;
-  if (n_rows <= 0) return;
-  if (bad && *bad) {
-    for (long long q = blockIdx.x * (long long)blockDim.x + threadIdx.x; q < q_hi - q_lo; q += (long long)gridDim.x * blockDim.x) keep_flag[q] = 0;
-    return;
-  }
-  for (long long chunk = warp; chunk < n_chunks; chunk += n_warps) {
-    const long long Q0 = q_lo + chunk * kSampleChunk;
-    const long long Q1 = Q0 + kSampleChunk < q_hi ? Q0 + kSampleChunk : q_hi;
-    long long base = warp_find_row(rp, n_rows, Q0, lane);
+  for (long long g = warp; g < d.chunk_off[d.n]; g += n_warps) {
+    const int i = prep_mat_of(d.chunk_off, d.n, g);
+    const PrepMat &M = d.mat[i];
+    const long long local = g - d.chunk_off[i];
+    const long long n_rows = M.n_rows, row_base = M.row_base;
+    const int32_t n_cols = M.n_cols, m = M.m;
+    const long long Q0 = M.q_lo + local * kSampleChunk;
+    const long long Q1 = Q0 + kSampleChunk < M.q_hi ? Q0 + kSampleChunk : M.q_hi;
+    uint32_t *keep = M.keep + local * kChunkWords;
+    if ((M.bad && *M.bad) || n_rows <= 0) {
+      if (lane < kChunkWords) keep[lane] = 0;
+      if (lane == 0) chunk_kept[g] = 0;
+      continue;
+    }
+    uint32_t n_kept = 0;
+    long long base = warp_find_row(M.rp, n_rows, Q0, lane);
     long long start_i, end_i;
     unsigned long long t_i, x_i;
     uint32_t kept_i;
@@ -54,23 +151,31 @@
     t_i = kKeepAlways;                                                                                      \
     x_i = 0;                                                                                                \
     if (r < n_rows) {                                                                                       \
-      start_i = rp[r];                                                                                      \
-      end_i = rp[r + 1];                                                                                    \
-      const long long d = end_i - start_i;                                                                  \
-      if (d > (long long)m) t_i = rate_threshold(row_sample_rate(d, m, intdiv));  \
+      start_i = M.rp[r];                                                                                    \
+      end_i = M.rp[r + 1];                                                                                  \
+      const long long dd = end_i - start_i;                                                                 \
+      if (dd > (long long)m) t_i = rate_threshold(row_sample_rate(dd, m, intdiv));  \
       x_i = mix64(((uint64_t)(uint32_t)seed << 32) | (uint64_t)(uint32_t)(row_base + r));                   \
     }                                                                                                       \
     kept_i = 0;                                                                                             \
   }
 #define CCO_FLUSH_WINDOW()                                                                                  \
-  if (kept_i) atomicAdd(&kept_per_row[row_base + base + lane], kept_i);
+  if (kept_i) atomicAdd(&M.kept_per_row[row_base + base + lane], kept_i);
     CCO_LOAD_WINDOW()
-    for (long long qb = Q0; qb < Q1; qb += 32) {
+    int w_end = kChunkWords;
+#pragma unroll
+    for (int w = 0; w < kChunkWords; ++w) {
+      const long long qb = Q0 + 32 * w;
+      if (qb >= Q1 || base >= n_rows) {
+        w_end = w;
+        break;
+      }
       const long long q = qb + lane;
       bool pending = q < Q1;
-      const int32_t j = pending ? col[q] : 0;
-      unsigned long long t_col = kKeepAlways;
-      if (pending && (uint32_t)j < (uint32_t)n_cols) t_col = col_thr[j];
+      const int32_t j = pending ? M.col[q] : 0;
+      const bool col_ok = pending && (uint32_t)j < (uint32_t)n_cols;
+      const unsigned long long t_col = col_ok ? M.col_thr[j] : kKeepAlways;
+      unsigned word = 0;
       while (true) {
         int idx = 0;
 #pragma unroll
@@ -87,13 +192,13 @@
         const unsigned long long x_row = __shfl_sync(0xffffffffu, x_i, src);
         const bool here = pending && idx < 32;
         const bool real_row = base + idx < n_rows;
-        bool keep = false;
+        bool keep_e = false;
         if (here) {
-          keep = real_row && (uint32_t)j < (uint32_t)n_cols && keep_entry_thr(t_row, t_col, x_row, (uint32_t)j);
-          keep_flag[q - q_lo] = keep ? 1 : 0;
-          if (keep && new_counts) atomicAdd(&new_counts[j], 1);
-        }
-        const unsigned kb = __ballot_sync(0xffffffffu, keep);
+          keep_e = real_row && col_ok && keep_entry_thr(t_row, t_col, x_row, (uint32_t)j);
+          if (keep_e && M.counts) atomicAdd(&M.counts[j], 1);
+        }
+        const unsigned kb = __ballot_sync(0xffffffffu, keep_e);
+        word |= kb;
         const int a = start_i <= qb ? 0 : (start_i >= qb + 32 ? 32 : (int)(start_i - qb));
         const int b = end_i <= qb ? 0 : (end_i >= qb + 32 ? 32 : (int)(end_i - qb));
         if (b > a) {
@@ -106,55 +211,81 @@
         CCO_FLUSH_WINDOW()
         base += 32;
         if (base >= n_rows) {
-          if (pending) keep_flag[q - q_lo] = 0;
           kept_i = 0;
           start_i = end_i = kNoRow;
           break;
         }
         CCO_LOAD_WINDOW()
       }
-      if (base >= n_rows) {
-        for (long long q2 = qb + 32 + lane; q2 < Q1; q2 += 32) keep_flag[q2 - q_lo] = 0;
-        break;
-      }
-    }
+      if (lane == 0) keep[w] = word;
+      n_kept += __popc(word);
+    }
+    if (lane >= w_end && lane < kChunkWords) keep[lane] = 0;
     if (base < n_rows && base + lane < n_rows) { CCO_FLUSH_WINDOW() }
+    if (lane == 0) chunk_kept[g] = n_kept;
 #undef CCO_LOAD_WINDOW
 #undef CCO_FLUSH_WINDOW
   }
 }
 
-__global__ void k_check_row_ptr(long long n_rows, const long long *__restrict__ rp, long long q_lo, long long q_hi, int *flags) {
-  int bad = 0;
-  for (long long r = blockIdx.x * (long long)blockDim.x + threadIdx.x; r < n_rows; r += (long long)gridDim.x * blockDim.x) {
-    const long long s = rp[r], e = rp[r + 1];
-    if (e < s || s < q_lo || e > q_hi) bad = 1;
-  }
-  if (bad) atomicOr(&flags[0], 1);
-}
-template <bool AGG>
-__global__ void k_col_histogram_flat(long long n, const int32_t *__restrict__ col, int32_t n_cols, int32_t *__restrict__ counts, int n_copies,
-                                     long long copy_stride, int *flags ) {
-  int32_t *mine = counts + (long long)(blockIdx.x % n_copies) * copy_stride;
+__global__ void __launch_bounds__(256) k_sample_write(const __grid_constant__ PrepMats d, const long long *__restrict__ chunk_pos) {
   const int lane = threadIdx.x & 31;
-  int bad = 0;
-  for (long long q0 = blockIdx.x * (long long)blockDim.x + (threadIdx.x & ~31); q0 < n; q0 += (long long)gridDim.x * blockDim.x) {
-    const long long q = q0 + lane;
-    const bool act = q < n;
-    const int32_t j = act ? col[q] : -1;
-    const bool ok = act && (uint32_t)j < (uint32_t)n_cols;
-    if (act && !ok) bad = 1;
-    if (AGG) {
-      const unsigned om = __ballot_sync(0xffffffffu, ok);
-      if (ok) {
-        const unsigned peers = __match_any_sync(om, j);
-        if ((__ffs(peers) - 1) == lane) atomicAdd(&mine[j], __popc(peers));
+  const long long warp = (blockIdx.x * (long long)blockDim.x + threadIdx.x) >> 5;
+  const long long n_warps = ((long long)gridDim.x * blockDim.x) >> 5;
+  const unsigned below = (1u << lane) - 1u;
+  for (long long g = warp; g < d.chunk_off[d.n]; g += n_warps) {
+    const int i = prep_mat_of(d.chunk_off, d.n, g);
+    const PrepMat &M = d.mat[i];
+    const long long local = g - d.chunk_off[i];
+    const long long Q0 = M.q_lo + local * kSampleChunk;
+    int32_t *out = M.dst + (chunk_pos[g] - chunk_pos[d.chunk_off[i]]);
+    const uint32_t mine = lane < kChunkWords ? M.keep[local * kChunkWords + lane] : 0u;
+#pragma unroll
+    for (int w = 0; w < kChunkWords; ++w) {
+      const unsigned word = __shfl_sync(0xffffffffu, mine, w);
+      const long long q = Q0 + w * 32 + lane;
+      if ((word >> lane) & 1u) out[__popc(word & below)] = M.col[q];
+      out += __popc(word);
+    }
+  }
+}
+
+__global__ void __launch_bounds__(256) k_transpose_scatter(long long n_rows, const uint32_t *__restrict__ rp, const int32_t *__restrict__ col,
+                                                           uint32_t *__restrict__ cursor, int32_t *__restrict__ users) {
+  const int lane = threadIdx.x & 31;
+  const long long warp = (blockIdx.x * (long long)blockDim.x + threadIdx.x) >> 5;
+  const long long n_warps = ((long long)gridDim.x * blockDim.x) >> 5;
+  if (n_rows <= 0) return;
+  const long long nnz = rp[n_rows];
+  const long long kNoRow = 0x7fffffffffffffffLL;
+  for (long long Q0 = warp * kSampleChunk; Q0 < nnz; Q0 += n_warps * kSampleChunk) {
+    const long long Q1 = Q0 + kSampleChunk < nnz ? Q0 + kSampleChunk : nnz;
+    long long base = warp_find_row(rp, n_rows, Q0, lane);
+    long long end_i = base + lane < n_rows ? (long long)rp[base + lane + 1] : kNoRow;
+    for (long long qb = Q0; qb < Q1; qb += 32) {
+      const long long q = qb + lane;
+      bool pending = q < Q1;
+      while (true) {
+        int idx = 0;
+#pragma unroll
+        for (int step = 16; step > 0; step >>= 1) {
+          const long long v = __shfl_sync(0xffffffffu, end_i, idx + step - 1);
+          if (v <= q) idx += step;
+        }
+        {
+          const long long v = __shfl_sync(0xffffffffu, end_i, idx);
+          if (v <= q) idx += 1;
+        }
+        if (pending && idx < 32) {
+          users[atomicAdd(&cursor[col[q]], 1u)] = (int32_t)(base + idx);
+          pending = false;
+        }
+        if (!__any_sync(0xffffffffu, pending)) break;
+        base += 32;
+        end_i = base + lane < n_rows ? (long long)rp[base + lane + 1] : kNoRow;
       }
-    } else if (ok) {
-      atomicAdd(&mine[j], 1);
-    }
-  }
-  if (flags && bad) atomicOr(&flags[0], 1);
-}
-
-}
+    }
+  }
+}
+
+}
```

Result: faster. 4.301 billion (median of 6 runs) (+3.6%).
